# hulop/SfM

Measured on AMD Instinct MI355X. Metric: BA iterations/sec + residual-evals/sec (cams x pts x obs); 1/2/4/8 GPU, higher is better.
Workload: dtype f64; 1 GPU; C3 per GPU: full BA solve (LM + DENSE_SCHUR, Ceres default options); cams=500, points=200000, observations=2000000, points_per_gpu=200000, obs_per_gpu=2000000, views_per_point=10, parallelism=single GPU, reduced_camera_factor=single GPU

## Files before the change

### sfm_amd/csrc/ba_device.h

```cpp
#pragma once
#include <hip/hip_runtime.h>
#include <algorithm>
#include <cstdint>

namespace sfm {

constexpr int kJRec = 20;
constexpr int kJX = 0, kRes = 6, kJC = 8;
constexpr int kEU = 4;
constexpr int kCamR = 36;
constexpr int kUcam = 28;
constexpr int kPtV = 10;
constexpr int kPtL = 10;
constexpr int kPtS = 16;
constexpr int kNB = 64;
constexpr int kThreads = 256;
constexpr uint32_t kYSentinelWord = 0x7FF4DEADu;
constexpr uint64_t kYSentinel = (uint64_t(kYSentinelWord) << 32) | kYSentinelWord;

enum Scalar {
  kCost = 0,
  kGradMaxCam,
  kGradMaxPt,
  kXNorm2Cam,
  kXNorm2Pt,
  kModelChange,
  kNewCost,
  kStep2Pt,
  kStep2Cam,
  kBadStep,
  kCholFail,
  kBadCam,
  kBadBack,
  kModelChangePt,
  kNumScalars
};

struct ReduceJob {
  int slot, nb, op, dst;
};
struct ReduceBatch {
  ReduceJob job[8];
  int n = 0;
  void add(int slot, int nb, int op, int dst) { job[n++] = ReduceJob{slot, nb, op, dst}; }
};

struct DevProblem {
  int32_t C = 0, P = 0;
  int64_t N = 0;
  int32_t* pt_off = nullptr;
  int32_t* order = nullptr;
  int64_t N_pad = 0;
  int32_t* cam_obs = nullptr;
  int32_t* cam_rng = nullptr;
  int32_t* cm_p = nullptr;
  int4* jchunks = nullptr;
  int32_t n_jchunks = 0;
  int32_t xcd_slice_max = 0;
  int32_t* tile_cnt = nullptr;
  int32_t* tile_exp = nullptr;
  int32_t overlap = 0;
  int32_t* jgrp = nullptr;
  int32_t jac_blocks = 1;
  int32_t jac_blocks_rec = 1;
  double* uv_cm = nullptr;
  int32_t* pos = nullptr;
  double* Kc = nullptr;
  double* cam = nullptr;
  double* cam_new = nullptr;
  double* X = nullptr;
  double* X_new = nullptr;
  double* cam0 = nullptr;
  double* X0 = nullptr;
  double* scale_c = nullptr;
  double* scale_p = nullptr;
  double* diag_c = nullptr;
  double* diag_p = nullptr;
  double* camR = nullptr;
  double* camRn = nullptr;
  double* jrec = nullptr;
  double* eu = nullptr;
  bool eu_cm = false;
  double* ypt = nullptr;
  int32_t* wcam = nullptr;
  double* ptV = nullptr;
  double* ptL = nullptr;
  double* Ucam = nullptr;
  int32_t n = 0, ld = 0, nblk = 0;
  double* S = nullptr;
  double* Spack = nullptr;
  double* invL = nullptr;
  double* ysol = nullptr;
  int32_t* fail = nullptr;
  int32_t* flags = nullptr;
  int32_t* cflags = nullptr;
  unsigned long long* cticket = nullptr;
  int32_t n_cu = 0;
  double min_diag = 1e-6, max_diag = 1e32;

  int64_t n_blk = 0, n_pairs = 0;
  int2* blk = nullptr;
  int32_t* seg = nullptr;
  int32_t* bpts = nullptr;
  int32_t* bperm = nullptr;
  int64_t n_bslots = 0;
  double* ptS = nullptr;
  int32_t schur_pts_sub = 8;
  bool schur_wg_blocks = false;
  double* dpart = nullptr;
  double* jpart = nullptr;
  double* uv_pm = nullptr;
  int32_t* cam_pm = nullptr;
  double* partials = nullptr;
  int32_t max_blocks = 0;
  double* scal = nullptr;
  double* scal_host = nullptr;
  const int32_t* gate = nullptr;
  const double* radius_dev = nullptr;
};

enum PartialSlot {
  kPCost = 0, kPXNormCam, kPXNormPt, kPGradCam, kPGradPt, kPModel, kPNewCost, kPStepPt, kPStepCam, kPBad,
  kPBadCam, kPBadBack, kPModelPt,
  kNumPartialSlots
};

void launch_cam_prep(const DevProblem& d, double* cam, bool count_norm, hipStream_t s);
void launch_cam_prep_accept(const DevProblem& d, bool count_norm, int grid, hipStream_t s);
void launch_jacobian(const DevProblem& d, bool scaled, hipStream_t s, bool write_records = false);
void launch_cam_reduce(const DevProblem& d, hipStream_t s);
void launch_cam_finalize(const DevProblem& d, int mode, bool reuse_diag, bool count_grad, hipStream_t s);
void launch_cam_sum_finalize(const DevProblem& d, int mode, bool count_grad, hipStream_t s);
void launch_point_eval(const DevProblem& d, int mode, bool reuse_diag, hipStream_t s);
void launch_point_prep(const DevProblem& d, double radius, hipStream_t s);
void launch_point_factor(const DevProblem& d, double radius, hipStream_t s);
void launch_schur(const DevProblem& d, double radius, bool add_diag, hipStream_t s);
void launch_schur_diag(const DevProblem& d, double radius, bool add_diag, hipStream_t s);
void launch_schur_offdiag(const DevProblem& d, int* tile_cnt, hipStream_t s);
void launch_pad_init(const DevProblem& d, hipStream_t s);
void launch_pack_upper(const DevProblem& d, bool unpack, hipStream_t s);
void launch_gated_copy(const double* src, double* dst, int64_t n, double scale, const int32_t* gate, hipStream_t s);
void launch_cam_update(const DevProblem& d, bool count_norm, hipStream_t s);
bool launch_point_eval_with_cams(const DevProblem& d, int mode, bool count_grad, hipStream_t s);
void launch_point_backsub(const DevProblem& d, hipStream_t s, bool cams_var = true, bool pts_var = true);
inline int obs_xcd_blocks(const DevProblem& d) {
  const int64_t per = d.xcd_slice_max > 0 ? (int64_t(d.xcd_slice_max) + 3) / 4
                                          : ((d.N_pad / 64 + 3) / 4 + 7) / 8;
  return int(8 * std::max<int64_t>(1, per));
}
inline int pt_xcd_blocks(const DevProblem& d) {
  const int64_t per_slice = (int64_t(d.P) + 7) / 8;
  return int(8 * std::max<int64_t>(1, (per_slice + kThreads - 1) / kThreads));
}
void launch_cam_solve(const DevProblem& d, double radius, hipStream_t s);
void launch_reduce(const DevProblem& d, int slot, int nb, int op, int dst, hipStream_t s);
void launch_reduce_batch(const DevProblem& d, const ReduceBatch& b, bool copy_fail, hipStream_t s);
int blocks_for(int64_t n, int threads);

bool launch_cholesky(const DevProblem& d, int epoch, hipStream_t s, bool clear_fail = true, int cam_step = -1,
                     int overlap = 0);
void launch_backsolve(const DevProblem& d, int epoch, hipStream_t s, bool sentinel_set = false);

int launch_cholesky_panel(const DevProblem& d, int k, int pt, int epoch, hipStream_t s);
void launch_panel_update(const DevProblem& d, int k, int j0, int j1, int pt, int nranks, int rank, hipStream_t s);
int panel_update_tiles(int nblk, int pt, int j0, int j1, int nranks, int rank);
constexpr int kPanelPack = 0, kPanelUnpack = 1, kPanelAdd = 2;
void launch_panel_copy(const DevProblem& d, int mode, int pt, int col0, int col1, const int64_t* off, int64_t off1,
                       double* buf, hipStream_t s);
void launch_fail_slot(const DevProblem& d, bool put, double* slot, hipStream_t s);
void launch_spd_fill(double* A, int ld, int n, unsigned seed, hipStream_t s);

}
```

### sfm_amd/csrc/ba_kernels.hip

```cpp
#include <hip/hip_runtime.h>
#include <cfloat>
#include <cmath>
#include <cstdlib>
#include "ba_device.h"
#include "ba_common.h"

namespace sfm {

namespace {

__global__ __launch_bounds__(kThreads) void k_cam_prep(int C, double* __restrict__ cam,
                                                       double* __restrict__ camR, double* __restrict__ part_xn, const int* __restrict__ gate,
                                                       const double* __restrict__ cam_src, const double* __restrict__ X_src,
                                                       double* __restrict__ X_dst, int64_t n_x) {
  if (gate && *gate == 0) return;
  __shared__ double sh[4];
  const int c = blockIdx.x * blockDim.x + threadIdx.x;
  for (int64_t i = int64_t(blockIdx.x) * blockDim.x + threadIdx.x; i < n_x; i += int64_t(gridDim.x) * blockDim.x)
    X_dst[i] = X_src[i];
  if (int64_t(blockIdx.x) * blockDim.x >= C) return;
  double xn = 0.0;
  if (c < C) {
    const double* cs = cam_src ? cam_src : cam;
    double x6[6];
// ... 122 lines not shown
    const double2 uv_nxt = ld2(uv_cm + 2 * (int64_t(ch_n.y) + l));
    const int p_nn = cm_p[int64_t(chunk_at(t + 2).y) + l];
    const double* cr = camR + size_t(kCamR) * c;
    const double* k = Kc + 5 * size_t(c);
    double sc[6];
#pragma unroll
    for (int a = 0; a < 6; ++a) sc[a] = scaled ? scale_c[6 * size_t(c) + a] : 1.0;
    {
      double rec[kJRec];
      const double cl = jac_record(cr, cam[6 * c + 3], cam[6 * c + 4], cam[6 * c + 5], k[0], k[1], k[2], k[3], k[4],
                                   sc, spc, Xc, uv_cur, rec);
      cost += (l < cnt) ? cl : 0.0;
      if (kRec) {
        double* mine = wst + l * kJRec;
#pragma unroll
        for (int f = 0; f < kJRec; f += 2) st2(mine + f, rec[f], rec[f + 1]);
      }
      if (jpart) {
        double j0[6], j1[6], r0 = rec[kRes], r1 = rec[kRes + 1];
#pragma unroll
        for (int a = 0; a < 6; ++a) {
          j0[a] = rec[kJC + a];
          j1[a] = rec[kJC + 6 + a];
        }
        if (cnt < 64) {
          const bool real = l < cnt;
#pragma unroll
          for (int a = 0; a < 6; ++a) {
            j0[a] = real ? j0[a] : 0.0;
            j1[a] = real ? j1[a] : 0.0;
          }
          r0 = real ? r0 : 0.0;
          r1 = real ? r1 : 0.0;
        }
        int q = 0;
#pragma unroll
        for (int a = 0; a < 6; ++a)
#pragma unroll
          for (int b = a; b < 6; ++b, ++q) acc[q] += j0[a] * j0[b] + j1[a] * j1[b];
#pragma unroll
        for (int a = 0; a < 6; ++a) acc[21 + a] += j0[a] * r0 + j1[a] * r1;
        double tot = 0.0;
        if (t + 1 >= n_chunks || ch_n.x != c) {
          tot = wave_sum32(acc, l);
#pragma unroll
          for (int e = 0; e < 32; ++e) acc[e] = 0.0;
        }
        if (!(l & 1) && (l >> 1) < 27) jpart[size_t(ib / 64) * 27 + (l >> 1)] = tot;
      }
    }
    if (kRec) {
      wave_lds_sync();
      jac_flush(wst, jrec, ib, l);
      wave_lds_sync();
    }
#pragma unroll
    for (int j = 0; j < 3; ++j) { Xc[j] = Xn[j]; spc[j] = spn[j]; }
    uv_cur = uv_nxt;
    p_nxt = p_nn;
  }
  const double r = block_reduce(cost, sh, false);
  if (threadIdx.x == 0) part_cost[blockIdx.x] = r;
}

__global__ __launch_bounds__(64) void k_cam_sum(const int32_t* __restrict__ cam_rng,
                                                const double* __restrict__ jpart, double* __restrict__ Ucam, const int* __restrict__ gate) {
  if (gate && *gate == 0) return;
  const int c = blockIdx.x, t = threadIdx.x;
  const int w0 = cam_rng[2 * c] / 64, w1 = (cam_rng[2 * c + 1] + 63) / 64;
  double v[32];
#pragma unroll
  for (int e = 0; e < 32; ++e) v[e] = 0.0;
  for (int w = w0 + t; w < w1; w += 64) {
    const double* src = jpart + size_t(w) * 27;
#pragma unroll
    for (int e = 0; e < 27; ++e) v[e] += src[e];
  }
  const double sum = wave_sum32(v, t);
  if (!(t & 1) && (t >> 1) < 27) Ucam[size_t(kUcam) * c + (t >> 1)] = sum;
}

struct CamFold {
  const int32_t* cam_rng;
  const double* jpart;
  double* Ucam;
  double* scale_c;
  double* diag_c;
  double min_diag, max_diag;
  int mode, C;
  double* part_grad;
};
__device__ __forceinline__ void cam_sum_body(int c, int t, const CamFold& f) {
  const int w0 = f.cam_rng[2 * c] / 64, w1 = (f.cam_rng[2 * c + 1] + 63) / 64;
  double v[32];
#pragma unroll
  for (int e = 0; e < 32; ++e) v[e] = 0.0;
  for (int w = w0 + t; w < w1; w += 64) {
    const double* src = f.jpart + size_t(w) * 27;
#pragma unroll
    for (int e = 0; e < 27; ++e) v[e] += src[e];
  }
  const double sum = wave_sum32(v, t);
  if (!(t & 1) && (t >> 1) < 27) f.Ucam[size_t(kUcam) * c + (t >> 1)] = sum;
  const int a = t < 6 ? t : 0;
  const double cn = __shfl(sum, 2 * up6(a, a)), ga = __shfl(sum, 2 * (21 + a));
  double g = 0.0;
  if (t < 6) {
    if (f.mode == 0) {
      f.scale_c[6 * c + a] = 1.0 / (1.0 + sqrt(cn));
    } else {
      f.diag_c[6 * c + a] = fmin(fmax(cn, f.min_diag), f.max_diag);
      g = fabs(ga / f.scale_c[6 * c + a]);
    }
  }
#pragma unroll
  for (int off = 4; off > 0; off >>= 1) g = fmax(g, __shfl_xor(g, off));
  if (t == 0 && f.part_grad) f.part_grad[c] = g;
}

__global__ __launch_bounds__(64) void k_cam_sum_finalize(const CamFold f, const int* __restrict__ gate) {
  if (gate && *gate == 0) return;
  cam_sum_body(blockIdx.x, threadIdx.x, f);
}

__global__ __launch_bounds__(kThreads) void k_cam_finalize(int C, const double* __restrict__ Ucam,
                                                           double* __restrict__ scale_c, double* __restrict__ diag_c,
                                                           double min_diag, double max_diag, int mode, int reuse,
                                                           double* __restrict__ part_grad, const int* __restrict__ gate) {
  if (gate && *gate == 0) return;
  __shared__ double sh[4];
  const int c = blockIdx.x * blockDim.x + threadIdx.x;
  double g = 0.0;
  if (c < C) {
    const double* U = Ucam + size_t(kUcam) * c;
    for (int a = 0; a < 6; ++a) {
      const double cn = U[up6(a, a)];
      if (mode == 0) {
        scale_c[6 * c + a] = 1.0 / (1.0 + sqrt(cn));
      } else {
        if (!reuse) diag_c[6 * c + a] = fmin(fmax(cn, min_diag), max_diag);
        g = fmax(g, fabs(U[21 + a] / scale_c[6 * c + a]));
      }
    }
  }
  const double r = block_reduce(g, sh, true);
  if (threadIdx.x == 0 && part_grad) part_grad[blockIdx.x] = r;
}

struct CamView {
  const double* R; const double* t; const double* K;
  int sR, sT, sK;
};

__device__ __forceinline__ void point_eval_body(int p, const int32_t* __restrict__ pt_off,
                                                const int32_t* __restrict__ cam_pm,
                                                const double* __restrict__ uv_pm, const CamView cv,
                                                const double* __restrict__ X, double* __restrict__ scale_p,
                                                double* __restrict__ diag_p, double* __restrict__ ptV,
                                                double min_diag, double max_diag, int mode, int reuse, double& g,
                                                double& xn) {
  double V[6] = {0, 0, 0, 0, 0, 0}, b[3] = {0, 0, 0};
  const double Xp[3] = {X[3 * size_t(p)], X[3 * size_t(p) + 1], X[3 * size_t(p) + 2]};
  double sp[3] = {1.0, 1.0, 1.0};
  if (mode == 1)
    for (int k = 0; k < 3; ++k) sp[k] = scale_p[3 * size_t(p) + k];
  const int q0 = pt_off[p], q1 = pt_off[p + 1];
  int c_n = q0 < q1 ? cam_pm[q0] : 0;
  double2 uv_n = q0 < q1 ? ld2(uv_pm + 2 * size_t(q0)) : make_double2(0.0, 0.0);
  for (int q = q0; q < q1; ++q) {
    const int c = c_n;
    const double2 uvo = uv_n;
    if (q + 1 < q1) {
      c_n = cam_pm[q + 1];
      uv_n = ld2(uv_pm + 2 * size_t(q + 1));
    }
    const double* cr = cv.R + size_t(cv.sR) * c;
    const double* k5 = cv.K + size_t(cv.sK) * c;
    const double* tc = cv.t + size_t(cv.sT) * c;
    const double fx = k5[0], sk = k5[1], cx = k5[2], fy = k5[3], cy = k5[4];
    const double pc0 = cr[0] * Xp[0] + cr[1] * Xp[1] + cr[2] * Xp[2] + tc[0];
    const double pc1 = cr[3] * Xp[0] + cr[4] * Xp[1] + cr[5] * Xp[2] + tc[1];
    const double pc2 = cr[6] * Xp[0] + cr[7] * Xp[1] + cr[8] * Xp[2] + tc[2];
    const SharedDiv dz = shared_div(pc2);
    const double xp = sdiv(dz, pc0), yp = sdiv(dz, pc1);
    const double r0 = fx * xp + sk * yp + cx - uvo.x;
    const double r1 = fy * yp + cy - uvo.y;
    const double iz = srcp(dz);
    const double a0 = fx * iz, a1 = sk * iz, a2 = -(fx * xp + sk * yp) * iz;
    const double b1 = fy * iz, b2 = -fy * yp * iz;
    double u[3], v[3];
#pragma unroll
    for (int j = 0; j < 3; ++j) {
      u[j] = (a0 * cr[j] + a1 * cr[3 + j] + a2 * cr[6 + j]) * sp[j];
      v[j] = (b1 * cr[3 + j] + b2 * cr[6 + j]) * sp[j];
    }
    V[0] += u[0] * u[0] + v[0] * v[0];
    V[1] += u[1] * u[0] + v[1] * v[0]; V[2] += u[1] * u[1] + v[1] * v[1];
    V[3] += u[2] * u[0] + v[2] * v[0]; V[4] += u[2] * u[1] + v[2] * v[1]; V[5] += u[2] * u[2] + v[2] * v[2];
    b[0] += u[0] * r0 + v[0] * r1; b[1] += u[1] * r0 + v[1] * r1; b[2] += u[2] * r0 + v[2] * r1;
  }
  const double cn[3] = {V[0], V[2], V[5]};
  if (mode == 0) {
    for (int k = 0; k < 3; ++k) scale_p[3 * size_t(p) + k] = 1.0 / (1.0 + sqrt(cn[k]));
  } else {
    for (int k = 0; k < 3; ++k) {
      if (!reuse) diag_p[3 * size_t(p) + k] = fmin(fmax(cn[k], min_diag), max_diag);
      g = fmax(g, fabs(b[k] / scale_p[3 * size_t(p) + k]));
      xn += X[3 * size_t(p) + k] * X[3 * size_t(p) + k];
    }
    double* o = ptV + size_t(kPtV) * p;
    st2(o, V[0], V[1]); st2(o + 2, V[2], V[3]); st2(o + 4, V[4], V[5]); st2(o + 6, b[0], b[1]); st2(o + 8, b[2], 0.0);
  }
}

__global__ __launch_bounds__(kThreads) void k_point_eval_rc(int P, const int32_t* __restrict__ pt_off,
                                                            const int32_t* __restrict__ cam_pm,
                                                            const double* __restrict__ uv_pm,
                                                            const double* __restrict__ camR,
                                                            const double* __restrict__ cam,
                                                            const double* __restrict__ Kc,
                                                            const double* __restrict__ X,
                                                            double* __restrict__ scale_p, double* __restrict__ diag_p,
                                                            double* __restrict__ ptV, double min_diag, double max_diag,
                                                            int mode, int reuse, double* __restrict__ part_grad,
                                                            double* __restrict__ part_xn, const int* __restrict__ gate) {
  if (gate && *gate == 0) return;
  __shared__ double sh[4];
  const int p = blockIdx.x * blockDim.x + threadIdx.x;
  double g = 0.0, xn = 0.0;
  if (p < P)
    point_eval_body(p, pt_off, cam_pm, uv_pm, CamView{camR, cam + 3, Kc, kCamR, 6, 5}, X, scale_p, diag_p, ptV,
                    min_diag, max_diag, mode, reuse, g, xn);
  if (mode == 1) {
    const double rg = block_reduce(g, sh, true);
    if (threadIdx.x == 0) part_grad[blockIdx.x] = rg;
    const double rx = block_reduce(xn, sh, false);
    if (threadIdx.x == 0) part_xn[blockIdx.x] = rx;
  }
}

constexpr int kCamE = 17;
template <int kMaxC, int kGroups = 1>
__global__ __launch_bounds__(kThreads * kGroups) void k_point_eval_lds(int P, int C, const int32_t* __restrict__ pt_off,
                                                             const int32_t* __restrict__ cam_pm,
                                                             const double* __restrict__ uv_pm,
                                                             const double* __restrict__ camR,
                                                             const double* __restrict__ cam,
                                                             const double* __restrict__ Kc,
                                                             const double* __restrict__ X,
                                                             double* __restrict__ scale_p, double* __restrict__ diag_p,
                                                             double* __restrict__ ptV, double min_diag, double max_diag,
                                                             int mode, int reuse, double* __restrict__ part_grad,
                                                             double* __restrict__ part_xn, const int* __restrict__ gate,
                                                             const CamFold cf) {
  if (gate && *gate == 0) return;
  static_assert(kGroups == 1 || kMaxC > 64, "the camera fold runs with one group per workgroup");
  const int nbp = (P + kThreads - 1) / kThreads;
  if (kGroups == 1 && int(blockIdx.x) >= nbp) {
    const int c = (int(blockIdx.x) - nbp) * (kThreads / 64) + int(threadIdx.x >> 6);
    if (c < cf.C) cam_sum_body(c, threadIdx.x & 63, cf);
    return;
  }
  __shared__ double sh[4 * kGroups];
  __shared__ double cst[kMaxC * kCamE];
  for (int i = threadIdx.x; i < C * kCamE; i += blockDim.x) {
    const int c = i / kCamE, j = i - c * kCamE;
    cst[i] = j < 9 ? camR[size_t(kCamR) * c + j] : j < 12 ? cam[6 * size_t(c) + 3 + (j - 9)] : Kc[5 * size_t(c) + (j - 12)];
  }
  __syncthreads();
  const int grp = int(threadIdx.x) / kThreads, tg = int(threadIdx.x) % kThreads;
  const int vb = int(blockIdx.x) * kGroups + grp;
  const int p = vb * kThreads + tg;
  double g = 0.0, xn = 0.0;
  if (p < P)
    point_eval_body(p, pt_off, cam_pm, uv_pm, CamView{cst, cst + 9, cst + 12, kCamE, kCamE, kCamE}, X, scale_p,
                    diag_p, ptV, min_diag, max_diag, mode, reuse, g, xn);
  if (mode == 1) {
    const int w = int(threadIdx.x) >> 6, l = int(threadIdx.x) & 63;
    const double wg = wave_max(g), wx = wave_sum(xn);
    if (l == 0) sh[w] = wg;
    __syncthreads();
    double rg = 0.0;
    if (tg == 0) {
      rg = sh[4 * grp];
      for (int i = 1; i < 4; ++i) rg = fmax(rg, sh[4 * grp + i]);
    }
    __syncthreads();
    if (l == 0) sh[w] = wx;
    __syncthreads();
    if (tg == 0 && vb < nbp) {
      double rx = sh[4 * grp];
      for (int i = 1; i < 4; ++i) rx = rx + sh[4 * grp + i];
      part_grad[vb] = rg;
      part_xn[vb] = rx;
    }
  }
}

__global__ __launch_bounds__(kThreads) void k_point_factor(int P, const double* __restrict__ ptV,
                                                           const double* __restrict__ diag_p, double radius,
                                                           double* __restrict__ ptL, double* __restrict__ part_bad,
                                                           const double* __restrict__ X,
                                                           const double* __restrict__ scale_p,
                                                           double* __restrict__ ptS, const int* __restrict__ gate, const double* __restrict__ radius_dev) {
  if (gate && *gate == 0) return;
  if (radius_dev) radius = *radius_dev;
  __shared__ double sh[4];
  const int p = blockIdx.x * blockDim.x + threadIdx.x;
  double bad = 0.0;
  if (p < P) {
    const double* v = ptV + size_t(kPtV) * p;
    double D[3];
    for (int k = 0; k < 3; ++k) { const double d = sqrt(diag_p[3 * size_t(p) + k] / radius); D[k] = d * d; }
    const double V00 = v[0] + D[0], V10 = v[1], V11 = v[2] + D[1], V20 = v[3], V21 = v[4], V22 = v[5] + D[2];
    const double l00 = sqrt(V00);
    const double l10 = V10 / l00, l20 = V20 / l00;
    const double l11 = sqrt(V11 - l10 * l10);
    const double l21 = (V21 - l20 * l10) / l11;
    const double l22 = sqrt(V22 - l20 * l20 - l21 * l21);
    if (!(l00 > 0.0) || !(l11 > 0.0) || !(l22 > 0.0)) bad = 1.0;
    const double z0 = v[6] / l00, z1 = (v[7] - l10 * z0) / l11, z2 = (v[8] - l20 * z0 - l21 * z1) / l22;
    double* L = ptL + size_t(kPtL) * p;
    st2(L, l00, l10); st2(L + 2, l11, l20); st2(L + 4, l21, l22); st2(L + 6, z0, z1); st2(L + 8, z2, 0.0);
    if (ptS) {
      double* o = ptS + size_t(kPtS) * p;
      const double* x = X + 3 * size_t(p);
      const double* sp = scale_p + 3 * size_t(p);
      st2(o, x[0], x[1]); st2(o + 2, x[2], sp[0]); st2(o + 4, sp[1], sp[2]);
      st2(o + 6, l10, l20); st2(o + 8, l21, 1.0 / l00); st2(o + 10, 1.0 / l11, 1.0 / l22);
      st2(o + 12, z0, z1); st2(o + 14, z2, 0.0);
    }
  }
  const double r = block_reduce(bad, sh, true);
  if (threadIdx.x == 0) part_bad[blockIdx.x] = r;
}

struct ObsRC {
  double rec[kJRec];
  double M[6];
  double h0, h1;
};
__device__ __forceinline__ void obs_recompute(int c, int p, double2 uvo, const double* __restrict__ camR,
                                              const double* __restrict__ cam, const double* __restrict__ Kc,
                                              const double* __restrict__ scale_c, const double* __restrict__ ptS,
                                              ObsRC& o) {
  const double* cr = camR + size_t(kCamR) * c;
  const double* k = Kc + 5 * size_t(c);
  const double* tc = cam + 6 * size_t(c) + 3;
  const double* sc = scale_c + 6 * size_t(c);
  const double fx = k[0], sk = k[1], cx = k[2], fy = k[3], cy = k[4];
  const double* rp = ptS + size_t(kPtS) * p;
  double q[16];
#pragma unroll
  for (int f = 0; f < 16; f += 2) {
    const double2 x = ld2(rp + f);
    q[f] = x.x; q[f + 1] = x.y;
  }
  const double Xp[3] = {q[0], q[1], q[2]}, sp[3] = {q[3], q[4], q[5]};
  const double pc0 = cr[0] * Xp[0] + cr[1] * Xp[1] + cr[2] * Xp[2] + tc[0];
  const double pc1 = cr[3] * Xp[0] + cr[4] * Xp[1] + cr[5] * Xp[2] + tc[1];
  const double pc2 = cr[6] * Xp[0] + cr[7] * Xp[1] + cr[8] * Xp[2] + tc[2];
  const double iz = srcp(shared_div(pc2)), xp = pc0 * iz, yp = pc1 * iz;
  double* rec = o.rec;
  rec[kRes] = fx * xp + sk * yp + cx - uvo.x;
  rec[kRes + 1] = fy * yp + cy - uvo.y;
  const double a0 = fx * iz, a1 = sk * iz, a2 = -(fx * xp + sk * yp) * iz;
  const double b1 = fy * iz, b2 = -fy * yp * iz;
#pragma unroll
  for (int j = 0; j < 3; ++j) {
    rec[kJX + j] = (a0 * cr[j] + a1 * cr[3 + j] + a2 * cr[6 + j]) * sp[j];
    rec[kJX + 3 + j] = (b1 * cr[3 + j] + b2 * cr[6 + j]) * sp[j];
  }
#pragma unroll
  for (int kk = 0; kk < 3; ++kk) {
    const double* D = cr + 9 + 9 * kk;
    const double q0 = D[0] * Xp[0] + D[1] * Xp[1] + D[2] * Xp[2];
    const double q1 = D[3] * Xp[0] + D[4] * Xp[1] + D[5] * Xp[2];
    const double q2 = D[6] * Xp[0] + D[7] * Xp[1] + D[8] * Xp[2];
    rec[kJC + kk] = (a0 * q0 + a1 * q1 + a2 * q2) * sc[kk];
    rec[kJC + 6 + kk] = (b1 * q1 + b2 * q2) * sc[kk];
  }
  rec[kJC + 3] = a0 * sc[3]; rec[kJC + 4] = a1 * sc[4]; rec[kJC + 5] = a2 * sc[5];
  rec[kJC + 9] = 0.0;        rec[kJC + 10] = b1 * sc[4]; rec[kJC + 11] = b2 * sc[5];
  const double l10 = q[6], l20 = q[7], l21 = q[8], i00 = q[9], i11 = q[10], i22 = q[11];
  const double* e = rec + kJX;
  o.M[0] = e[0] * i00; o.M[1] = (e[1] - l10 * o.M[0]) * i11; o.M[2] = (e[2] - l20 * o.M[0] - l21 * o.M[1]) * i22;
  o.M[3] = e[3] * i00; o.M[4] = (e[4] - l10 * o.M[3]) * i11; o.M[5] = (e[5] - l20 * o.M[3] - l21 * o.M[4]) * i22;
  o.h0 = o.M[0] * q[12] + o.M[1] * q[13] + o.M[2] * q[14];
  o.h1 = o.M[3] * q[12] + o.M[4] * q[13] + o.M[5] * q[14];
}

struct XcdChunks {
  int t, end, stride;
};
__device__ __forceinline__ XcdChunks xcd_chunks(const int32_t* __restrict__ grp_off, int wv) {
  const int grp = blockIdx.x & 7;
  const int nbg = (int(gridDim.x) - 1 - grp) / 8 + 1;
  const int wi = (blockIdx.x >> 3) * (kThreads / 64) + wv;
  return XcdChunks{grp_off[grp] + wi, grp_off[grp + 1], nbg * (kThreads / 64)};
}

__global__ __launch_bounds__(kThreads) void k_obs_prep_rc(const int32_t* __restrict__ grp_off,
                                                          const int4* __restrict__ chunks,
                                                          const int32_t* __restrict__ cm_p,
                                                          const double* __restrict__ uv_cm,
                                                          const int32_t* __restrict__ cam_obs,
                                                          const double* __restrict__ camR,
                                                          const double* __restrict__ cam,
                                                          const double* __restrict__ Kc,
                                                          const double* __restrict__ scale_c,
                                                          const double* __restrict__ ptS,
                                                          double* __restrict__ dpart, const int* __restrict__ gate) {
  if (gate && *gate == 0) return;
  const int l = threadIdx.x & 63, wv = threadIdx.x >> 6;
  const XcdChunks xc = xcd_chunks(grp_off, wave_uniform(wv));
  if (xc.t >= xc.end) return;
  const int4 ch = chunks[xc.t];
  const int64_t i0 = __builtin_amdgcn_readfirstlane(ch.y);
  const int64_t i = i0 + l;
  const int c = __builtin_amdgcn_readfirstlane(ch.x);
  ObsRC o;
  obs_recompute(c, cm_p[i], ld2(uv_cm + 2 * i), camR, cam, Kc, scale_c, ptS, o);
  const double* jc = o.rec + kJC;
  double F[18];
#pragma unroll
  for (int u = 0; u < 6; ++u) {
    F[3 * u] = jc[u] * o.M[0] + jc[6 + u] * o.M[3];
    F[3 * u + 1] = jc[u] * o.M[1] + jc[6 + u] * o.M[4];
    F[3 * u + 2] = jc[u] * o.M[2] + jc[6 + u] * o.M[5];
  }
  double r0 = o.rec[kRes] - o.h0, r1 = o.rec[kRes + 1] - o.h1;
  if (__builtin_amdgcn_readfirstlane(ch.z) < 64) {
    const bool real = cam_obs[i] >= 0;
#pragma unroll
    for (int e = 0; e < 18; ++e) F[e] = real ? F[e] : 0.0;
    r0 = real ? r0 : 0.0;
    r1 = real ? r1 : 0.0;
  }
  double v[32];
  int q = 0;
#pragma unroll
  for (int u = 0; u < 6; ++u)
#pragma unroll
    for (int w = u; w < 6; ++w, ++q)
      v[q] = F[3 * u] * F[3 * w] + F[3 * u + 1] * F[3 * w + 1] + F[3 * u + 2] * F[3 * w + 2];
#pragma unroll
  for (int u = 0; u < 6; ++u) v[21 + u] = jc[u] * r0 + jc[6 + u] * r1;
#pragma unroll
  for (int e = 27; e < 32; ++e) v[e] = 0.0;
  const double tot = wave_sum32(v, l);
  if (!(l & 1) && (l >> 1) < 27) dpart[size_t(i0 / 64) * 27 + (l >> 1)] = tot;
}

__global__ __launch_bounds__(kThreads) void k_backsub_a_rc(const int32_t* __restrict__ grp_off,
                                                           const int4* __restrict__ chunks,
                                                           const int32_t* __restrict__ cm_p,
                                                           const double* __restrict__ uv_cm,
                                                           const int32_t* __restrict__ cam_obs,
                                                           const double* __restrict__ camR,
                                                           const double* __restrict__ cam,
                                                           const double* __restrict__ Kc,
                                                           const double* __restrict__ scale_c,
                                                           const double* __restrict__ ptS,
                                                           const double* __restrict__ ysol, double* __restrict__ eu,
                                                           int eu_cm, double* __restrict__ part_model, const int* __restrict__ gate) {
  if (gate && *gate == 0) return;
  __shared__ double sh[4];
  const int l = threadIdx.x & 63, wv = threadIdx.x >> 6;
  double model = 0.0;
  const XcdChunks xc = xcd_chunks(grp_off, wave_uniform(wv));
  for (int t = xc.t; t < xc.end; t += xc.stride) {
    const int4 ch = chunks[t];
    const int64_t i = int64_t(__builtin_amdgcn_readfirstlane(ch.y)) + l;
    const int c = __builtin_amdgcn_readfirstlane(ch.x);
    ObsRC o;
    obs_recompute(c, cm_p[i], ld2(uv_cm + 2 * i), camR, cam, Kc, scale_c, ptS, o);
    const double* y = ysol + 6 * size_t(c);
    const double* J = o.rec + kJC;
    double e0 = 0.0, e1 = 0.0;
#pragma unroll
    for (int k = 0; k < 6; ++k) { e0 += J[k] * y[k]; e1 += J[6 + k] * y[k]; }
    const int qo = cam_obs[i];
    if (qo >= 0) {
      model += e0 * o.rec[kRes] + e1 * o.rec[kRes + 1] - 0.5 * (e0 * e0 + e1 * e1);
      const double* M = o.M;
      double* dst = eu + 4 * (eu_cm ? size_t(i) : size_t(qo));
      st2(dst, M[0] * e0 + M[3] * e1, M[1] * e0 + M[4] * e1);
      st2(dst + 2, M[2] * e0 + M[5] * e1, 0.0);
    }
  }
  const double r = block_reduce(model, sh, false);
  if (threadIdx.x == 0) part_model[blockIdx.x] = r;
}

__device__ __forceinline__ void schur_diag_body(int c, int C, int t, const int32_t* __restrict__ cam_rng,
                                                const double* __restrict__ dpart, const double* __restrict__ Ucam,
                                                const double* __restrict__ diag_c, double radius, int add_diag,
                                                double* __restrict__ S, int ld, int n, int init,
                                                int* __restrict__ fail, unsigned long long* __restrict__ ysol,
                                                int n_y) {
  for (int j = 6 * c; j < 6 * c + 6; ++j) {
    for (int i = n + 1 + t; i < ld; i += 64) S[size_t(j) * ld + i] = 0.0;
    if (t == 0 && j < n_y) ysol[j] = kYSentinel;
  }
  if (c == C - 1) {
    for (int j = n; j < ld; ++j) {
      for (int i = (j > n ? j : n + 1) + t; i < ld; i += 64) S[size_t(j) * ld + i] = (i == j) ? 1.0 : 0.0;
      if (t == 0 && j < n_y) ysol[j] = kYSentinel;
    }
    if (t == 0) {
      S[size_t(n) * ld + n] = 1.0;
      *fail = 0;
    }
  }
  const int w0 = cam_rng[2 * c] / 64, w1 = (cam_rng[2 * c + 1] + 63) / 64;
  double v[32];
#pragma unroll
  for (int e = 0; e < 32; ++e) v[e] = 0.0;
  for (int w = w0 + t; w < w1; w += 64) {
    const double* src = dpart + size_t(w) * 27;
#pragma unroll
    for (int e = 0; e < 27; ++e) v[e] += src[e];
  }
  const double sum = wave_sum32(v, t);
  const int tu = t < 36 ? t / 6 : 0, tv = t < 36 ? t % 6 : 0;
  const int src = t < 36 ? up6(tu, tv) : (t < 42 ? 21 + (t - 36) : 0);
  const double tot = __shfl(sum, 2 * src);
  if (t < 36) {
    const int u = tu, vv = tv, q = src;
    double* sp = S + size_t(6 * c + u) * ld + 6 * size_t(c) + vv;
    double val = (init ? 0.0 : *sp) - tot;
    if (add_diag) {
      val += Ucam[size_t(kUcam) * c + q];
      if (u == vv) { const double dd = sqrt(diag_c[6 * size_t(c) + u] / radius); val += dd * dd; }
    }
    *sp = val;
  } else if (t < 42) {
    S[size_t(6 * c + (t - 36)) * ld + n] = tot;
  }
}

struct DiagFold {
  const int32_t* cam_rng;
  const double* dpart;
  const double* Ucam;
  const double* diag_c;
  double radius;
  const double* radius_dev;
  int add_diag, C, n, n_y;
  int* fail;
  unsigned long long* ysol;
};

constexpr int kCamS = 50;

__device__ __forceinline__ void stage_cam(double* cs, int c, const double* __restrict__ camR,
                                          const double* __restrict__ cam, const double* __restrict__ Kc,
                                          const double* __restrict__ scale_c, int l) {
  if (l < 36) cs[l] = camR[size_t(kCamR) * c + l];
  else if (l < 39) cs[l] = cam[6 * size_t(c) + 3 + (l - 36)];
  else if (l < 44) cs[l] = Kc[5 * size_t(c) + (l - 39)];
  else if (l < 50) cs[l] = scale_c[6 * size_t(c) + (l - 44)];
}

__device__ __forceinline__ void pair_side_m(const double* cs, const double Xp[3], const double sp[3],
                                            const double Lp[6], double M[6], double ab[5]) {
  const double* cr = cs;
  const double fx = cs[39], sk = cs[40], fy = cs[42];
  const double pc0 = cr[0] * Xp[0] + cr[1] * Xp[1] + cr[2] * Xp[2] + cs[36];
  const double pc1 = cr[3] * Xp[0] + cr[4] * Xp[1] + cr[5] * Xp[2] + cs[37];
  const double pc2 = cr[6] * Xp[0] + cr[7] * Xp[1] + cr[8] * Xp[2] + cs[38];
  const double iz = srcp(shared_div(pc2)), xp = pc0 * iz, yp = pc1 * iz;
  const double a0 = fx * iz, a1 = sk * iz, a2 = -(fx * xp + sk * yp) * iz;
  const double b1 = fy * iz, b2 = -fy * yp * iz;
  ab[0] = a0; ab[1] = a1; ab[2] = a2; ab[3] = b1; ab[4] = b2;
  double e[6];
#pragma unroll
  for (int j = 0; j < 3; ++j) {
    e[j] = (a0 * cr[j] + a1 * cr[3 + j] + a2 * cr[6 + j]) * sp[j];
    e[3 + j] = (b1 * cr[3 + j] + b2 * cr[6 + j]) * sp[j];
  }
  const double l10 = Lp[0], l20 = Lp[1], l21 = Lp[2], i00 = Lp[3], i11 = Lp[4], i22 = Lp[5];
  M[0] = e[0] * i00; M[1] = (e[1] - l10 * M[0]) * i11; M[2] = (e[2] - l20 * M[0] - l21 * M[1]) * i22;
  M[3] = e[3] * i00; M[4] = (e[4] - l10 * M[3]) * i11; M[5] = (e[5] - l20 * M[3] - l21 * M[4]) * i22;
}
template <int kSub>
__device__ __forceinline__ void seg_reduce32(double (&v)[32], int l) {
#pragma unroll
  for (int d = (kSub >= 64 ? 32 : kSub / 2), n = 32; d >= 1 && n > 1; d >>= 1, n >>= 1) {
    const int h = n / 2;
    const uint64_t m = (l & d) ? ~0ull : 0ull;
#pragma unroll
    for (int j = 0; j < h; ++j) {
      const uint64_t a = __builtin_bit_cast(uint64_t, v[j]), b = __builtin_bit_cast(uint64_t, v[h + j]);
      const double keep = __builtin_bit_cast(double, (b & m) | (a & ~m));
      const double send = __builtin_bit_cast(double, (a & m) | (b & ~m));
      v[j] = keep + __shfl_xor(send, d);
    }
  }
  if (kSub == 64) v[0] += __shfl_xor(v[0], 1);
}
template <int kSub>
__device__ __forceinline__ double seg_sum(double v) {
#pragma unroll
  for (int off = kSub / 2; off > 0; off >>= 1) v += __shfl_xor(v, off);
  return v;
}

template <int kSub, int kWpb = 1>
__global__ __launch_bounds__(kThreads, 3) void k_schur_pts(int64_t n_slots, const int2* __restrict__ blk,
                                                        const int32_t* __restrict__ seg,
                                                        const int32_t* __restrict__ bpts,
                                                        const double* __restrict__ ptS,
                                                        const double* __restrict__ camR,
                                                        const double* __restrict__ cam, const double* __restrict__ Kc,
                                                        const double* __restrict__ scale_c, double* __restrict__ S,
                                                        int ld,
                                                        const int32_t* __restrict__ bperm, const int* __restrict__ gate,
                                                        int* __restrict__ tile_cnt, int nbt, const DiagFold df) {
  if (gate && *gate == 0) return;
  static_assert(kWpb == 1 || (kWpb == kThreads / 64 && kSub == 64), "4 waves per block take 64 lanes each");
  constexpr int kPer = 64 / kSub;
  __shared__ __attribute__((aligned(16))) double cst[kThreads / 64][kPer][2 * kCamS];
  const int l = threadIdx.x & 63, wv = threadIdx.x >> 6, g = l / kSub, sl = l % kSub;
  const int64_t wb = kWpb == 1 ? (int64_t(blockIdx.x) * (kThreads / 64) + wv) * kPer : int64_t(blockIdx.x);
  constexpr int kStride = kSub * kWpb;
  const int lane0 = kWpb == 1 ? sl : 64 * wv + sl;
  auto slot_blk = [&](int64_t k) -> int32_t { return k < n_slots ? (bperm ? bperm[k] : int32_t(k)) : -1; };
  const int32_t bs = slot_blk(wb + g);
  const bool own = bs >= 0;
  const int64_t b = own ? bs : 0;
  const int2 cc = blk[b];
  double* cs1 = cst[wv][g];
  double* cs2 = cs1 + kCamS;
#pragma unroll
  for (int q = 0; q < kPer; ++q) {
    const int32_t bq = slot_blk(wb + q);
    const int2 cq = blk[bq >= 0 ? bq : 0];
    stage_cam(cst[wv][q], cq.x, camR, cam, Kc, scale_c, l);
    stage_cam(cst[wv][q] + kCamS, cq.y, camR, cam, Kc, scale_c, l);
  }
  wave_lds_sync();
  if (kWpb > 1 && df.C > 0 && own && cc.x == cc.y && wv == 0) {
    const double radius = df.radius_dev ? *df.radius_dev : df.radius;
    schur_diag_body(cc.x, df.C, l, df.cam_rng, df.dpart, df.Ucam, df.diag_c, radius, df.add_diag, S, ld, df.n, 1,
                    df.fail, df.ysol, df.n_y);
    asm volatile("s_waitcnt vmcnt(0)" ::: "memory");
  }
  const int kb = seg[b], ke = own ? seg[b + 1] : kb;
  double acc[36];
#pragma unroll
  for (int e = 0; e < 36; ++e) acc[e] = 0.0;
  int len = ke - kb;
#pragma unroll
  for (int off = kSub; off < 64; off <<= 1) len = max(len, __shfl_xor(len, off));
  int p_nx = bpts[kb + lane0 < ke ? kb + lane0 : 0];
  for (int k0 = 0; k0 < len; k0 += kStride) {
    asm volatile("" ::: "memory");
    const int k = kb + k0 + lane0;
    const bool valid = k < ke;
    const int p = p_nx;
    p_nx = bpts[k + kStride < ke ? k + kStride : 0];
    const double* r = ptS + size_t(kPtS) * p;
    double q[12];
#pragma unroll
    for (int f = 0; f < 12; f += 2) {
      const double2 x = ld2(r + f);
      q[f] = x.x; q[f + 1] = x.y;
    }
    const double Xp[3] = {q[0], q[1], q[2]}, sp[3] = {q[3], q[4], q[5]};
    const double Lp[6] = {q[6], q[7], q[8], q[9], q[10], q[11]};
    double M1[6], ab1[5], M2[6], ab2[5];
    pair_side_m(cs1, Xp, sp, Lp, M1, ab1);
    pair_side_m(cs2, Xp, sp, Lp, M2, ab2);
    asm volatile("" ::: "memory");
    const double w = valid ? 1.0 : 0.0;
    const double g00 = (M1[0] * M2[0] + M1[1] * M2[1] + M1[2] * M2[2]) * w;
    const double g01 = (M1[0] * M2[3] + M1[1] * M2[4] + M1[2] * M2[5]) * w;
    const double g10 = (M1[3] * M2[0] + M1[4] * M2[1] + M1[5] * M2[2]) * w;
    const double g11 = (M1[3] * M2[3] + M1[4] * M2[4] + M1[5] * M2[5]) * w;
    double H[3][3];
    {
      const double t00 = g00 * ab2[0], t01 = g00 * ab2[1] + g01 * ab2[3], t02 = g00 * ab2[2] + g01 * ab2[4];
      const double t10 = g10 * ab2[0], t11 = g10 * ab2[1] + g11 * ab2[3], t12 = g10 * ab2[2] + g11 * ab2[4];
      H[0][0] = ab1[0] * t00; H[0][1] = ab1[0] * t01; H[0][2] = ab1[0] * t02;
      H[1][0] = ab1[1] * t00 + ab1[3] * t10; H[1][1] = ab1[1] * t01 + ab1[3] * t11; H[1][2] = ab1[1] * t02 + ab1[3] * t12;
      H[2][0] = ab1[2] * t00 + ab1[4] * t10; H[2][1] = ab1[2] * t01 + ab1[4] * t11; H[2][2] = ab1[2] * t02 + ab1[4] * t12;
    }
    double HQ[3][3];
#pragma unroll
    for (int k = 0; k < 3; ++k) {
      const double* D = cs2 + 9 + 9 * k;
      const double q0 = D[0] * Xp[0] + D[1] * Xp[1] + D[2] * Xp[2];
      const double q1 = D[3] * Xp[0] + D[4] * Xp[1] + D[5] * Xp[2];
      const double q2 = D[6] * Xp[0] + D[7] * Xp[1] + D[8] * Xp[2];
#pragma unroll
      for (int i = 0; i < 3; ++i) HQ[i][k] = H[i][0] * q0 + H[i][1] * q1 + H[i][2] * q2;
    }
#pragma unroll
    for (int u = 0; u < 3; ++u) {
      const double* D = cs1 + 9 + 9 * u;
      const double q0 = D[0] * Xp[0] + D[1] * Xp[1] + D[2] * Xp[2];
      const double q1 = D[3] * Xp[0] + D[4] * Xp[1] + D[5] * Xp[2];
      const double q2 = D[6] * Xp[0] + D[7] * Xp[1] + D[8] * Xp[2];
#pragma unroll
      for (int v = 0; v < 3; ++v) {
        acc[6 * u + v] += q0 * HQ[0][v] + q1 * HQ[1][v] + q2 * HQ[2][v];
        acc[6 * u + 3 + v] += q0 * H[0][v] + q1 * H[1][v] + q2 * H[2][v];
      }
    }
#pragma unroll
    for (int u = 0; u < 3; ++u)
#pragma unroll
      for (int v = 0; v < 3; ++v) {
        acc[6 * (3 + u) + v] += HQ[u][v];
        acc[6 * (3 + u) + 3 + v] += H[u][v];
      }
  }
  double v32[32];
#pragma unroll
  for (int e = 0; e < 32; ++e) v32[e] = acc[e];
  seg_reduce32<kSub>(v32, l);
  double t32 = seg_sum<kSub>(acc[32]), t33 = seg_sum<kSub>(acc[33]), t34 = seg_sum<kSub>(acc[34]),
         t35 = seg_sum<kSub>(acc[35]);
  if (kWpb > 1) {
    __shared__ double red[kWpb][36];
    if (!(sl & 1)) red[wv][sl >> 1] = v32[0];
    if (sl == 0) { red[wv][32] = t32; red[wv][33] = t33; red[wv][34] = t34; red[wv][35] = t35; }
    __syncthreads();
    if (wv != 0) return;
    if (!(sl & 1)) {
      double a = red[0][sl >> 1];
#pragma unroll
      for (int q = 1; q < kWpb; ++q) a += red[q][sl >> 1];
      v32[0] = a;
    }
    if (sl < 4) {
      double a = red[0][32 + sl];
#pragma unroll
      for (int q = 1; q < kWpb; ++q) a += red[q][32 + sl];
      if (sl == 0) t32 = a; else if (sl == 1) t33 = a; else if (sl == 2) t34 = a; else t35 = a;
    }
  }
  if (own) {
    double* Sb = S + size_t(6 * cc.x) * ld + 6 * size_t(cc.y);
    const bool add = cc.x == cc.y;
    const double* sc1 = cst[wv][g] + 44;
    const double* sc2 = sc1 + kCamS;
    auto put = [&](int e, double v) {
      double* q = Sb + size_t(e / 6) * ld + e % 6;
      v = v * sc1[e / 6] * sc2[e % 6];
      v = add ? *q - v : -v;
      if (tile_cnt) __hip_atomic_store(q, v, __ATOMIC_RELAXED, __HIP_MEMORY_SCOPE_AGENT);
      else *q = v;
    };
    constexpr int kR = kSub >= 32 ? 1 : 32 / kSub;
    if (kSub == 64) {
      if (!(sl & 1)) put(sl >> 1, v32[0]);
    } else {
#pragma unroll
      for (int r = 0; r < kR; ++r) put(kR * sl + r, v32[r]);
    }
    if (sl < 4) put(32 + sl, sl == 0 ? t32 : sl == 1 ? t33 : sl == 2 ? t34 : t35);
  }
  if (tile_cnt) {
    asm volatile("s_waitcnt vmcnt(0)" ::: "memory");
    if (own && sl == 0) {
      const int r0 = 6 * cc.y, c0 = 6 * cc.x;
      for (int I = r0 / 64; I <= (r0 + 5) / 64; ++I)
        for (int J = c0 / 64; J <= (c0 + 5) / 64; ++J)
          __hip_atomic_fetch_add(tile_cnt + I * nbt + J, 1, __ATOMIC_RELAXED, __HIP_MEMORY_SCOPE_AGENT);
    }
  }
}

template <int kSub, int kHalf>
__global__ __launch_bounds__(kThreads, 4) void k_schur_pts_half(int64_t n_slots, const int2* __restrict__ blk,
                                                             const int32_t* __restrict__ seg,
                                                             const int32_t* __restrict__ bpts,
                                                             const double* __restrict__ ptS,
                                                             const double* __restrict__ camR,
                                                             const double* __restrict__ cam,
                                                             const double* __restrict__ Kc,
                                                             const double* __restrict__ scale_c, double* __restrict__ S,
                                                             int ld, const int32_t* __restrict__ bperm,
                                                             const int* __restrict__ gate) {
  if (gate && *gate == 0) return;
  constexpr int kPer = 64 / kSub;
  __shared__ __attribute__((aligned(16))) double cst[kThreads / 64][kPer][2 * kCamS];
  const int l = threadIdx.x & 63, wv = threadIdx.x >> 6, g = l / kSub, sl = l % kSub;
  const int64_t wb = (int64_t(blockIdx.x) * (kThreads / 64) + wv) * kPer;
  auto slot_blk = [&](int64_t k) -> int32_t { return k < n_slots ? (bperm ? bperm[k] : int32_t(k)) : -1; };
  const int32_t bs = slot_blk(wb + g);
  const bool own = bs >= 0;
  const int64_t b = own ? bs : 0;
  const int2 cc = blk[b];
  double* cs1 = cst[wv][g];
  double* cs2 = cs1 + kCamS;
#pragma unroll
  for (int q = 0; q < kPer; ++q) {
    const int32_t bq = slot_blk(wb + q);
    const int2 cq = blk[bq >= 0 ? bq : 0];
    stage_cam(cst[wv][q], cq.x, camR, cam, Kc, scale_c, l);
    stage_cam(cst[wv][q] + kCamS, cq.y, camR, cam, Kc, scale_c, l);
  }
  wave_lds_sync();
  const int kb = seg[b], ke = own ? seg[b + 1] : kb;
  double acc[18];
#pragma unroll
  for (int e = 0; e < 18; ++e) acc[e] = 0.0;
  int len = ke - kb;
#pragma unroll
  for (int off = kSub; off < 64; off <<= 1) len = max(len, __shfl_xor(len, off));
  int p_nx = bpts[kb + sl < ke ? kb + sl : 0];
  for (int k0 = 0; k0 < len; k0 += kSub) {
    asm volatile("" ::: "memory");
    const int k = kb + k0 + sl;
    const bool valid = k < ke;
    const int p = p_nx;
    p_nx = bpts[k + kSub < ke ? k + kSub : 0];
    const double* r = ptS + size_t(kPtS) * p;
    double q[12];
#pragma unroll
    for (int f = 0; f < 12; f += 2) {
      const double2 x = ld2(r + f);
      q[f] = x.x; q[f + 1] = x.y;
    }
    const double Xp[3] = {q[0], q[1], q[2]}, sp[3] = {q[3], q[4], q[5]};
    const double Lp[6] = {q[6], q[7], q[8], q[9], q[10], q[11]};
    double M1[6], ab1[5], M2[6], ab2[5];
    pair_side_m(cs1, Xp, sp, Lp, M1, ab1);
    pair_side_m(cs2, Xp, sp, Lp, M2, ab2);
    asm volatile("" ::: "memory");
    const double w = valid ? 1.0 : 0.0;
    const double g00 = (M1[0] * M2[0] + M1[1] * M2[1] + M1[2] * M2[2]) * w;
    const double g01 = (M1[0] * M2[3] + M1[1] * M2[4] + M1[2] * M2[5]) * w;
    const double g10 = (M1[3] * M2[0] + M1[4] * M2[1] + M1[5] * M2[2]) * w;
    const double g11 = (M1[3] * M2[3] + M1[4] * M2[4] + M1[5] * M2[5]) * w;
    double H[3][3];
    {
      const double t00 = g00 * ab2[0], t01 = g00 * ab2[1] + g01 * ab2[3], t02 = g00 * ab2[2] + g01 * ab2[4];
      const double t10 = g10 * ab2[0], t11 = g10 * ab2[1] + g11 * ab2[3], t12 = g10 * ab2[2] + g11 * ab2[4];
      H[0][0] = ab1[0] * t00; H[0][1] = ab1[0] * t01; H[0][2] = ab1[0] * t02;
      H[1][0] = ab1[1] * t00 + ab1[3] * t10; H[1][1] = ab1[1] * t01 + ab1[3] * t11; H[1][2] = ab1[1] * t02 + ab1[3] * t12;
      H[2][0] = ab1[2] * t00 + ab1[4] * t10; H[2][1] = ab1[2] * t01 + ab1[4] * t11; H[2][2] = ab1[2] * t02 + ab1[4] * t12;
    }
    double HQ[3][3];
#pragma unroll
    for (int kq = 0; kq < 3; ++kq) {
      const double* D = cs2 + 9 + 9 * kq;
      const double q0 = D[0] * Xp[0] + D[1] * Xp[1] + D[2] * Xp[2];
      const double q1 = D[3] * Xp[0] + D[4] * Xp[1] + D[5] * Xp[2];
      const double q2 = D[6] * Xp[0] + D[7] * Xp[1] + D[8] * Xp[2];
#pragma unroll
      for (int i = 0; i < 3; ++i) HQ[i][kq] = H[i][0] * q0 + H[i][1] * q1 + H[i][2] * q2;
    }
    if (kHalf == 0) {
#pragma unroll
      for (int u = 0; u < 3; ++u) {
        const double* D = cs1 + 9 + 9 * u;
        const double q0 = D[0] * Xp[0] + D[1] * Xp[1] + D[2] * Xp[2];
        const double q1 = D[3] * Xp[0] + D[4] * Xp[1] + D[5] * Xp[2];
        const double q2 = D[6] * Xp[0] + D[7] * Xp[1] + D[8] * Xp[2];
#pragma unroll
        for (int v = 0; v < 3; ++v) {
          acc[6 * u + v] += q0 * HQ[0][v] + q1 * HQ[1][v] + q2 * HQ[2][v];
          acc[6 * u + 3 + v] += q0 * H[0][v] + q1 * H[1][v] + q2 * H[2][v];
        }
      }
    } else {
#pragma unroll
      for (int u = 0; u < 3; ++u)
#pragma unroll
        for (int v = 0; v < 3; ++v) {
          acc[6 * u + v] += HQ[u][v];
          acc[6 * u + 3 + v] += H[u][v];
        }
    }
  }
  double v32[32];
#pragma unroll
  for (int e = 0; e < 32; ++e) v32[e] = e < 18 ? acc[e] : 0.0;
  seg_reduce32<kSub>(v32, l);
  if (own) {
    double* Sb = S + size_t(6 * cc.x) * ld + 6 * size_t(cc.y);
    const bool add = cc.x == cc.y;
    const double* sc1 = cst[wv][g] + 44;
    const double* sc2 = sc1 + kCamS;
    auto put = [&](int e, double v) {
      double* q = Sb + size_t(e / 6) * ld + e % 6;
      v = v * sc1[e / 6] * sc2[e % 6];
      *q = add ? *q - v : -v;
    };
    constexpr int kR = kSub >= 32 ? 1 : 32 / kSub;
    if (kSub == 64) {
      if (!(sl & 1) && (sl >> 1) < 18) put(18 * kHalf + (sl >> 1), v32[0]);
    } else {
#pragma unroll
      for (int r = 0; r < kR; ++r)
        if (kR * sl + r < 18) put(18 * kHalf + kR * sl + r, v32[r]);
    }
  }
}

__global__ __launch_bounds__(64) void k_schur_diag_sum(const int32_t* __restrict__ cam_rng,
                                                       const double* __restrict__ dpart,
                                                       const double* __restrict__ Ucam,
                                                       const double* __restrict__ diag_c, double radius,
                                                       int add_diag, double* __restrict__ S, int ld, int n,
                                                       int init, const int* __restrict__ gate, const double* __restrict__ radius_dev,
                                                       int* __restrict__ fail, unsigned long long* __restrict__ ysol, int n_y) {
  if (gate && *gate == 0) return;
  if (radius_dev) radius = *radius_dev;
  schur_diag_body(blockIdx.x, gridDim.x, threadIdx.x, cam_rng, dpart, Ucam, diag_c, radius, add_diag, S, ld, n, init,
                  fail, ysol, n_y);
}

__device__ __forceinline__ size_t packed_row(int i, int n) { return size_t(i) * (n + 1) - size_t(i) * (i - 1) / 2; }

__global__ void k_pack_upper(const double* __restrict__ S, int ld, int n, double* __restrict__ P, const int* __restrict__ gate) {
  if (gate && *gate == 0) return;
  const int i = blockIdx.x;
  const double* row = S + size_t(i) * ld;
  double* dst = P + packed_row(i, n) - i;
  for (int j = i + threadIdx.x; j <= n; j += blockDim.x) dst[j] = row[j];
}

__global__ void k_unpack_upper(const double* __restrict__ P, int ld, int n, double* __restrict__ S, const int* __restrict__ gate) {
  if (gate && *gate == 0) return;
  const int i = blockIdx.x;
  double* row = S + size_t(i) * ld;
  const double* src = P + packed_row(i, n) - i;
  for (int j = i + threadIdx.x; j <= n; j += blockDim.x) row[j] = src[j];
}

__global__ void k_gated_copy(const double* src, double* dst, int64_t n, double scale, const int* __restrict__ gate) {
  if (gate && *gate == 0) return;
  for (int64_t i = blockIdx.x * int64_t(blockDim.x) + threadIdx.x; i < n; i += int64_t(gridDim.x) * blockDim.x)
    dst[i] = src[i] * scale;
}

__global__ void k_pad_init(double* __restrict__ S, int ld, int n, int* __restrict__ fail,
                           unsigned long long* __restrict__ ysol, int n_y, const int* __restrict__ gate) {
  if (gate && *gate == 0) return;
  const int j = blockIdx.x;
  if (j == 0 && threadIdx.x == 0) *fail = 0;
  if (threadIdx.x == 0 && j < n_y) ysol[j] = kYSentinel;
  for (int i = (j > n ? j : n + 1) + threadIdx.x; i < ld; i += blockDim.x) S[size_t(j) * ld + i] = (i == j) ? 1.0 : 0.0;
  if (j == n && threadIdx.x == 0) S[size_t(n) * ld + n] = 1.0;
}

__global__ __launch_bounds__(kThreads) void k_cam_update(int C, const double* __restrict__ cam,
                                                         const double* __restrict__ ysol,
                                                         const double* __restrict__ scale_c,
                                                         double* __restrict__ cam_new, double* __restrict__ camRn,
                                                         double* __restrict__ part_step, double* __restrict__ part_bad, const int* __restrict__ gate) {
  if (gate && *gate == 0) return;
  __shared__ double sh[4];
  const int c = blockIdx.x * blockDim.x + threadIdx.x;
  double st = 0.0, bad = 0.0;
  if (c < C) cam_update_one(c, cam, ysol, scale_c, cam_new, camRn, st, bad);
  const double rs = block_reduce(st, sh, false);
  if (threadIdx.x == 0 && part_step) part_step[blockIdx.x] = rs;
  const double rb = block_reduce(bad, sh, true);
  if (threadIdx.x == 0) part_bad[blockIdx.x] = rb;
}

__global__ __launch_bounds__(kThreads) void k_cam_solve(int C, const double* __restrict__ Ucam,
                                                        const double* __restrict__ diag_c, double radius,
                                                        double* __restrict__ ysol, int* __restrict__ fail, const int* __restrict__ gate, const double* __restrict__ radius_dev) {
  if (gate && *gate == 0) return;
  if (radius_dev) radius = *radius_dev;
  const int c = blockIdx.x * blockDim.x + threadIdx.x;
  if (c >= C) return;
  const double* U = Ucam + size_t(kUcam) * c;
  double L[21], y[6];
  bool ok = true;
#pragma unroll
  for (int j = 0; j < 6; ++j) {
    double s = U[up6(j, j)] + diag_c[6 * c + j] / radius;
#pragma unroll
    for (int k = 0; k < j; ++k) s -= L[up6(k, j)] * L[up6(k, j)];
    ok = ok && s > 0.0 && isfinite(s);
    const double ljj = sqrt(s);
    L[up6(j, j)] = ljj;
#pragma unroll
    for (int i = j + 1; i < 6; ++i) {
      double a = U[up6(j, i)];
#pragma unroll
      for (int k = 0; k < j; ++k) a -= L[up6(k, i)] * L[up6(k, j)];
      L[up6(j, i)] = a / ljj;
    }
  }
#pragma unroll
  for (int i = 0; i < 6; ++i) {
    double s = U[21 + i];
#pragma unroll
    for (int k = 0; k < i; ++k) s -= L[up6(k, i)] * y[k];
    y[i] = s / L[up6(i, i)];
  }
#pragma unroll
  for (int i = 5; i >= 0; --i) {
    double s = y[i];
#pragma unroll
    for (int k = i + 1; k < 6; ++k) s -= L[up6(i, k)] * y[k];
    y[i] = s / L[up6(i, i)];
  }
#pragma unroll
  for (int i = 0; i < 6; ++i) ysol[6 * c + i] = y[i];
  if (!ok) atomicOr(fail, 1);
}


__global__ __launch_bounds__(kThreads) void k_backsub_b(int P, const int32_t* __restrict__ pt_off,
                                                        const double* __restrict__ eu,
                                                        const int32_t* __restrict__ eu_pos,
                                                        const double* __restrict__ ptL,
                                                        const double* __restrict__ ptV,
                                                        const double* __restrict__ scale_p,
                                                        const double* __restrict__ X, double* __restrict__ X_new,
                                                        double* __restrict__ ypt, double* __restrict__ part_step,
                                                        double* __restrict__ part_bad,
                                                        double* __restrict__ part_model, const int* __restrict__ gate) {
  if (gate && *gate == 0) return;
  __shared__ double sh[4];
  const int x = blockIdx.x & 7;
  const int pb = int((int64_t(x) * P + 7) / 8), pe = int((int64_t(x + 1) * P + 7) / 8);
  const int p = pb + (blockIdx.x >> 3) * blockDim.x + threadIdx.x;
  double st = 0.0, bad = 0.0, model = 0.0;
  if (p < pe) {
    const double* L = ptL + size_t(kPtL) * p;
    const double l00 = L[0], l10 = L[1], l11 = L[2], l20 = L[3], l21 = L[4], l22 = L[5];
    double w0 = L[6], w1 = L[7], w2 = L[8];
    double s0 = 0.0, s1 = 0.0, s2 = 0.0;
    const int q0 = pt_off[p], q1 = pt_off[p + 1];
    int q = q0;
    for (; q + 4 <= q1; q += 4) {
      int ps[4];
#pragma unroll
      for (int j = 0; j < 4; ++j) ps[j] = eu_pos ? eu_pos[q + j] : q + j;
      double2 a[4];
      double b[4];
#pragma unroll
      for (int j = 0; j < 4; ++j) {
        const double* u = eu + 4 * size_t(ps[j]);
        a[j] = ld2(u);
        b[j] = u[2];
      }
#pragma unroll
      for (int j = 0; j < 4; ++j) {
        w0 -= a[j].x;
        w1 -= a[j].y;
        w2 -= b[j];
        s0 += a[j].x; s1 += a[j].y; s2 += b[j];
      }
    }
    for (; q < q1; ++q) {
      const double* u = eu + 4 * (eu_pos ? size_t(eu_pos[q]) : size_t(q));
      const double2 u01 = ld2(u);
      const double u2 = u[2];
      w0 -= u01.x;
      w1 -= u01.y;
      w2 -= u2;
      s0 += u01.x; s1 += u01.y; s2 += u2;
    }
    const double y2 = w2 / l22;
    const double y1 = (w1 - l21 * y2) / l11;
    const double y0 = (w0 - l10 * y1 - l20 * y2) / l00;
    if (!isfinite(y0) || !isfinite(y1) || !isfinite(y2)) bad = 1.0;
    {
      const double* v = ptV + size_t(kPtV) * p;
      const double h0 = l00 * s0, h1 = l10 * s0 + l11 * s1, h2 = l20 * s0 + l21 * s1 + l22 * s2;
      const double yVy = v[0] * y0 * y0 + v[2] * y1 * y1 + v[5] * y2 * y2 +
                         2.0 * (v[1] * y0 * y1 + v[3] * y0 * y2 + v[4] * y1 * y2);
      model = y0 * (v[6] - h0) + y1 * (v[7] - h1) + y2 * (v[8] - h2) - 0.5 * yVy;
    }
    const double yp[3] = {y0, y1, y2};
    for (int k = 0; k < 3; ++k) {
      const double x = X[3 * size_t(p) + k];
      const double xn = x + scale_p[3 * size_t(p) + k] * (-yp[k]);
      const double d = x - xn;
      st += d * d;
      X_new[3 * size_t(p) + k] = xn;
      ypt[3 * size_t(p) + k] = yp[k];
    }
  }
  double r = block_reduce(st, sh, false);
  if (threadIdx.x == 0) part_step[blockIdx.x] = r;
  r = block_reduce(bad, sh, true);
  if (threadIdx.x == 0) part_bad[blockIdx.x] = r;
  r = block_reduce(model, sh, false);
  if (threadIdx.x == 0) part_model[blockIdx.x] = r;
}

__global__ __launch_bounds__(kThreads) void k_backsub_c(const int32_t* __restrict__ grp_off,
                                                        const int4* __restrict__ chunks,
                                                        const int32_t* __restrict__ cam_obs,
                                                        const int32_t* __restrict__ cm_p,
                                                        const double* __restrict__ uv_cm,
                                                        const double* __restrict__ Kc,
                                                        const double* __restrict__ X_new,
                                                        const double* __restrict__ camRn,
                                                        double* __restrict__ part_cost, const int* __restrict__ gate) {
  if (gate && *gate == 0) return;
  __shared__ double sh[4];
  const int l = threadIdx.x & 63, wv = threadIdx.x >> 6;
  const XcdChunks xc = xcd_chunks(grp_off, wave_uniform(wv));
  double ncost = 0.0;
  if (xc.t < xc.end) {
    const int4 ch = chunks[xc.t];
    const int64_t i = int64_t(__builtin_amdgcn_readfirstlane(ch.y)) + l;
    const int c = __builtin_amdgcn_readfirstlane(ch.x);
    const bool real = cam_obs[i] >= 0;
    const int p = cm_p[i];
    const double* Rn = camRn + 12 * size_t(c);
    const double Xn0 = X_new[3 * size_t(p)], Xn1 = X_new[3 * size_t(p) + 1], Xn2 = X_new[3 * size_t(p) + 2];
    double pc[3];
#pragma unroll
    for (int k = 0; k < 3; ++k) pc[k] = Rn[3 * k] * Xn0 + Rn[3 * k + 1] * Xn1 + Rn[3 * k + 2] * Xn2 + Rn[9 + k];
    const SharedDiv dz = shared_div(pc[2]);
    const double xp = sdiv(dz, pc[0]), ypj = sdiv(dz, pc[1]);
    const double* k5 = Kc + 5 * size_t(c);
    const double2 uvo = ld2(uv_cm + 2 * i);
    const double rn0 = k5[0] * xp + k5[1] * ypj + k5[2] - uvo.x;
    const double rn1 = k5[3] * ypj + k5[4] - uvo.y;
    if (real) ncost = 0.5 * (rn0 * rn0 + rn1 * rn1);
  }
  const double r = block_reduce(ncost, sh, false);
  if (threadIdx.x == 0) part_cost[blockIdx.x] = r;
}

__global__ __launch_bounds__(1024) void k_reduce_batch(const double* __restrict__ partials, int64_t max_blocks,
                                                       ReduceBatch b, double* __restrict__ scal,
                                                       const int* __restrict__ fail, const int* __restrict__ gate) {
  if (gate && *gate == 0) return;
  __shared__ double sh[16];
  reduce_batch_job(partials, max_blocks, b.job[blockIdx.x], scal, blockIdx.x == 0 ? fail : nullptr, sh);
}

__global__ __launch_bounds__(1024) void k_reduce(const double* __restrict__ src, int nb, int op,
                                                 double* __restrict__ dst) {
  __shared__ double sh[16];
  double v = 0.0;
  for (int i = threadIdx.x; i < nb; i += 1024) v = op ? fmax(v, src[i]) : v + src[i];
  v = op ? wave_max(v) : wave_sum(v);
  const int w = threadIdx.x >> 6, l = threadIdx.x & 63;
  if (l == 0) sh[w] = v;
  __syncthreads();
  if (threadIdx.x == 0) {
    double r = sh[0];
    for (int i = 1; i < 16; ++i) r = op ? fmax(r, sh[i]) : r + sh[i];
    *dst = r;
  }
}

}

int blocks_for(int64_t n, int threads) { return int((n + threads - 1) / threads); }

static inline double* slot(const DevProblem& d, int s) { return d.partials + size_t(s) * d.max_blocks; }

void launch_cam_prep(const DevProblem& d, double* cam, bool count_norm, hipStream_t s) {
  k_cam_prep<<<blocks_for(d.C, kThreads), kThreads, 0, s>>>(d.C, cam, d.camR, count_norm ? slot(d, kPXNormCam) : nullptr, d.gate,
                                                            nullptr, nullptr, nullptr, 0);
}
void launch_cam_prep_accept(const DevProblem& d, bool count_norm, int grid, hipStream_t s) {
  k_cam_prep<<<std::max(grid, blocks_for(d.C, kThreads)), kThreads, 0, s>>>(
      d.C, d.cam, d.camR, count_norm ? slot(d, kPXNormCam) : nullptr, d.gate, d.cam_new, d.X_new, d.X, 3 * int64_t(d.P));
}
void launch_jacobian(const DevProblem& d, bool scaled, hipStream_t s, bool write_records) {
  if (write_records)
    k_jacobian<true><<<d.jac_blocks_rec, kThreads, 0, s>>>(d.jgrp, d.jchunks, d.cm_p, d.uv_cm, d.Kc, d.cam, d.camR,
                                                           d.X, d.scale_c, d.scale_p, scaled ? 1 : 0, d.jrec,
                                                           slot(d, kPCost), d.jpart, d.gate);
  else
    k_jacobian<false><<<d.jac_blocks, kThreads, 0, s>>>(d.jgrp, d.jchunks, d.cm_p, d.uv_cm, d.Kc, d.cam, d.camR, d.X,
                                                        d.scale_c, d.scale_p, scaled ? 1 : 0, d.jrec, slot(d, kPCost),
                                                        d.jpart, d.gate);
}
void launch_cam_reduce(const DevProblem& d, hipStream_t s) {
  if (d.C) k_cam_sum<<<d.C, 64, 0, s>>>(d.cam_rng, d.jpart, d.Ucam, d.gate);
}
static CamFold cam_fold(const DevProblem& d, int mode, bool count_grad) {
  return CamFold{d.cam_rng, d.jpart, d.Ucam, d.scale_c, d.diag_c, d.min_diag, d.max_diag, mode, d.C,
                 count_grad ? slot(d, kPGradCam) : nullptr};
}
void launch_cam_sum_finalize(const DevProblem& d, int mode, bool count_grad, hipStream_t s) {
  if (d.C) k_cam_sum_finalize<<<d.C, 64, 0, s>>>(cam_fold(d, mode, count_grad), d.gate);
}
bool launch_point_eval_with_cams(const DevProblem& d, int mode, bool count_grad, hipStream_t s) {
  if (d.P == 0 || d.C == 0 || d.C > 64) return false;
  const int nb = blocks_for(d.P, kThreads) + (d.C + kThreads / 64 - 1) / (kThreads / 64);
  k_point_eval_lds<64><<<nb, kThreads, 0, s>>>(d.P, d.C, d.pt_off, d.cam_pm, d.uv_pm, d.camR, d.cam, d.Kc, d.X,
                                               d.scale_p, d.diag_p, d.ptV, d.min_diag, d.max_diag, mode, 0,
                                               slot(d, kPGradPt), slot(d, kPXNormPt), d.gate,
                                               cam_fold(d, mode, count_grad));
  return true;
}
void launch_cam_finalize(const DevProblem& d, int mode, bool reuse_diag, bool count_grad, hipStream_t s) {
  k_cam_finalize<<<blocks_for(d.C, kThreads), kThreads, 0, s>>>(d.C, d.Ucam, d.scale_c, d.diag_c, d.min_diag, d.max_diag, mode,
                                                               reuse_diag ? 1 : 0,
                                                               count_grad ? slot(d, kPGradCam) : nullptr, d.gate);
}
static bool env_flag_k(const char* name) {
  const char* v = std::getenv(name);
  return v && v[0] == '1';
}
void launch_point_eval(const DevProblem& d, int mode, bool reuse_diag, hipStream_t s) {
  if (d.P == 0) return;
  const int nb = blocks_for(d.P, kThreads);
#define SFM_PE_LDS(M_)                                                                                              \
  k_point_eval_lds<M_><<<nb, kThreads, 0, s>>>(d.P, d.C, d.pt_off, d.cam_pm, d.uv_pm, d.camR, d.cam, d.Kc, d.X,      \
                                               d.scale_p, d.diag_p, d.ptV, d.min_diag, d.max_diag, mode,           \
                                               reuse_diag ? 1 : 0, slot(d, kPGradPt), slot(d, kPXNormPt), d.gate,    \
                                               CamFold{})
  if (d.C <= 64) SFM_PE_LDS(64);
  else if (d.C <= 512 && !env_flag_k("SFM_PE_GROUPS1"))
    k_point_eval_lds<512, 2><<<blocks_for(d.P, 2 * kThreads), 2 * kThreads, 0, s>>>(
        d.P, d.C, d.pt_off, d.cam_pm, d.uv_pm, d.camR, d.cam, d.Kc, d.X, d.scale_p, d.diag_p, d.ptV, d.min_diag,
        d.max_diag, mode, reuse_diag ? 1 : 0, slot(d, kPGradPt), slot(d, kPXNormPt), d.gate, CamFold{});
  else if (d.C <= 512) SFM_PE_LDS(512);
  else
    k_point_eval_rc<<<nb, kThreads, 0, s>>>(d.P, d.pt_off, d.cam_pm, d.uv_pm, d.camR, d.cam, d.Kc, d.X, d.scale_p,
                                            d.diag_p, d.ptV, d.min_diag, d.max_diag, mode, reuse_diag ? 1 : 0,
                                            slot(d, kPGradPt), slot(d, kPXNormPt), d.gate);
#undef SFM_PE_LDS
}
void launch_point_factor(const DevProblem& d, double radius, hipStream_t s) {
  if (d.P) k_point_factor<<<blocks_for(d.P, kThreads), kThreads, 0, s>>>(d.P, d.ptV, d.diag_p, radius, d.ptL,
                                                                         slot(d, kPBad), d.X, d.scale_p, d.ptS, d.gate, d.radius_dev);
}
void launch_point_prep(const DevProblem& d, double radius, hipStream_t s) {
  launch_point_factor(d, radius, s);
  if (d.N_pad)
    k_obs_prep_rc<<<obs_xcd_blocks(d), kThreads, 0, s>>>(d.jgrp, d.jchunks, d.cm_p, d.uv_cm, d.cam_obs, d.camR, d.cam,
                                                         d.Kc, d.scale_c, d.ptS, d.dpart, d.gate);
}
void launch_schur(const DevProblem& d, double radius, bool add_diag, hipStream_t s) {
  if (d.schur_wg_blocks && d.n_blk && d.C) {
    const DiagFold f{d.cam_rng, d.dpart, d.Ucam, d.diag_c, radius, d.radius_dev, add_diag ? 1 : 0, d.C, d.n,
                     (d.n + kNB - 1) / kNB * kNB, d.fail, reinterpret_cast<unsigned long long*>(d.ysol)};
    k_schur_pts<64, kThreads / 64><<<int(d.n_bslots), kThreads, 0, s>>>(d.n_bslots, d.blk, d.seg, d.bpts, d.ptS,
                                                                       d.camR, d.cam, d.Kc, d.scale_c, d.S, d.ld,
                                                                       d.bperm, d.gate, nullptr, d.nblk, f);
    return;
  }
  launch_schur_diag(d, radius, add_diag, s);
  launch_schur_offdiag(d, nullptr, s);
}
void launch_schur_diag(const DevProblem& d, double radius, bool add_diag, hipStream_t s) {
  if (d.C)
    k_schur_diag_sum<<<d.C, 64, 0, s>>>(d.cam_rng, d.dpart, d.Ucam, d.diag_c, radius, add_diag ? 1 : 0, d.S, d.ld,
                                        d.n, 1, d.gate, d.radius_dev, d.fail,
                                        reinterpret_cast<unsigned long long*>(d.ysol), (d.n + kNB - 1) / kNB * kNB);
}
void launch_schur_offdiag(const DevProblem& d, int* tile_cnt, hipStream_t s) {
  if (!d.n_blk) return;
  const int64_t n_slots = tile_cnt ? d.n_blk : d.n_bslots;
  const int32_t* bperm = tile_cnt ? nullptr : d.bperm;
  const int sub = d.schur_pts_sub, per = 64 / sub * (kThreads / 64);
  const int nb = int((n_slots + per - 1) / per);
#define SFM_PTS(S_)                                                                                           \
  k_schur_pts<S_><<<nb, kThreads, 0, s>>>(n_slots, d.blk, d.seg, d.bpts, d.ptS, d.camR, d.cam, d.Kc, d.scale_c, \
                                          d.S, d.ld, bperm, d.gate, tile_cnt, d.nblk, DiagFold{})
  if (d.schur_wg_blocks) {
    k_schur_pts<64, kThreads / 64><<<int(n_slots), kThreads, 0, s>>>(n_slots, d.blk, d.seg, d.bpts, d.ptS,
                                                                    d.camR, d.cam, d.Kc, d.scale_c, d.S, d.ld,
                                                                    bperm, d.gate, tile_cnt, d.nblk, DiagFold{});
    return;
  }
  static const bool halves = [] {
    const char* e = std::getenv("SFM_SCHUR_HALVES");
    return e && e[0] == '1';
  }();
  if (halves && !tile_cnt) {
#define SFM_PTS_H(S_, H_)                                                                                       \
  k_schur_pts_half<S_, H_><<<nb, kThreads, 0, s>>>(n_slots, d.blk, d.seg, d.bpts, d.ptS, d.camR, d.cam, d.Kc, \
                                                   d.scale_c, d.S, d.ld, bperm, d.gate)
    if (sub == 8) { SFM_PTS_H(8, 0); SFM_PTS_H(8, 1); }
    else if (sub == 16) { SFM_PTS_H(16, 0); SFM_PTS_H(16, 1); }
    else if (sub == 32) { SFM_PTS_H(32, 0); SFM_PTS_H(32, 1); }
    else { SFM_PTS_H(64, 0); SFM_PTS_H(64, 1); }
#undef SFM_PTS_H
    return;
  }
  if (sub == 8) SFM_PTS(8);
  else if (sub == 16) SFM_PTS(16);
  else if (sub == 32) SFM_PTS(32);
  else SFM_PTS(64);
#undef SFM_PTS
}
void launch_pack_upper(const DevProblem& d, bool unpack, hipStream_t s) {
  if (d.n == 0) return;
  if (unpack) k_unpack_upper<<<d.n, 256, 0, s>>>(d.Spack, d.ld, d.n, d.S, d.gate);
  else k_pack_upper<<<d.n, 256, 0, s>>>(d.S, d.ld, d.n, d.Spack, d.gate);
}
void launch_gated_copy(const double* src, double* dst, int64_t n, double scale, const int32_t* gate, hipStream_t s) {
  if (n <= 0) return;
  const int grid = int(std::min<int64_t>(1024, (n + 255) / 256));
  k_gated_copy<<<grid, 256, 0, s>>>(src, dst, n, scale, gate);
}
void launch_pad_init(const DevProblem& d, hipStream_t s) {
  const int n_y = (d.n + kNB - 1) / kNB * kNB;
  k_pad_init<<<d.ld, 64, 0, s>>>(d.S, d.ld, d.n, d.fail, reinterpret_cast<unsigned long long*>(d.ysol), n_y, d.gate);
}
void launch_cam_update(const DevProblem& d, bool count_norm, hipStream_t s) {
  k_cam_update<<<blocks_for(d.C, kThreads), kThreads, 0, s>>>(d.C, d.cam, d.ysol, d.scale_c, d.cam_new, d.camRn,
                                                             count_norm ? slot(d, kPStepCam) : nullptr,
                                                             slot(d, kPBadCam), d.gate);
}
void launch_cam_solve(const DevProblem& d, double radius, hipStream_t s) {
  (void)hipMemsetAsync(d.fail, 0, sizeof(int), s);
  if (d.C) k_cam_solve<<<blocks_for(d.C, kThreads), kThreads, 0, s>>>(d.C, d.Ucam, d.diag_c, radius, d.ysol, d.fail, d.gate, d.radius_dev);
}
void launch_point_backsub(const DevProblem& d, hipStream_t s, bool cams_var, bool pts_var) {
  if (d.N_pad && cams_var)
    k_backsub_a_rc<<<obs_xcd_blocks(d), kThreads, 0, s>>>(d.jgrp, d.jchunks, d.cm_p, d.uv_cm, d.cam_obs, d.camR,
                                                          d.cam, d.Kc, d.scale_c, d.ptS, d.ysol, d.eu, d.eu_cm ? 1 : 0,
                                                          slot(d, kPModel), d.gate);
  else if (d.N_pad) {
    (void)hipMemsetAsync(d.eu, 0, sizeof(double) * 4 * size_t(d.eu_cm ? d.N_pad : d.N), s);
    (void)hipMemsetAsync(slot(d, kPModel), 0, sizeof(double) * size_t(obs_xcd_blocks(d)), s);
  }
  if (d.P && pts_var) {
    k_backsub_b<<<pt_xcd_blocks(d), kThreads, 0, s>>>(d.P, d.pt_off, d.eu, d.eu_cm ? d.pos : nullptr,
                                                               d.ptL, d.ptV, d.scale_p,
                                                               d.X, d.X_new, d.ypt, slot(d, kPStepPt),
                                                               slot(d, kPBadBack), slot(d, kPModelPt), d.gate);
  } else if (d.P) {
    const size_t nbP = size_t(pt_xcd_blocks(d));
    (void)hipMemsetAsync(d.ypt, 0, sizeof(double) * 3 * size_t(d.P), s);
    (void)hipMemcpyAsync(d.X_new, d.X, sizeof(double) * 3 * size_t(d.P), hipMemcpyDeviceToDevice, s);
    (void)hipMemsetAsync(slot(d, kPStepPt), 0, sizeof(double) * nbP, s);
    (void)hipMemsetAsync(slot(d, kPBadBack), 0, sizeof(double) * nbP, s);
    (void)hipMemsetAsync(slot(d, kPModelPt), 0, sizeof(double) * nbP, s);
  }
  if (d.N_pad)
    k_backsub_c<<<obs_xcd_blocks(d), kThreads, 0, s>>>(d.jgrp, d.jchunks, d.cam_obs, d.cm_p, d.uv_cm, d.Kc, d.X_new,
                                                       d.camRn, slot(d, kPNewCost), d.gate);
}
void launch_reduce(const DevProblem& d, int sl, int nb, int op, int dst, hipStream_t s) {
  k_reduce<<<1, 1024, 0, s>>>(slot(d, sl), nb, op, d.scal + dst);
}
void launch_reduce_batch(const DevProblem& d, const ReduceBatch& b, bool copy_fail, hipStream_t s) {
  if (b.n > 0)
    k_reduce_batch<<<b.n, 1024, 0, s>>>(d.partials, d.max_blocks, b, d.scal, copy_fail ? d.fail : nullptr, d.gate);
}

}
```

### sfm_amd/csrc/ba_solver.hip

```cpp
#include <hip/hip_runtime.h>
#include <rccl/rccl.h>
#include <map>
#include <atomic>
#include <thread>

#include <algorithm>
#include <array>
#include <cfloat>
#include <cmath>
#include <cstdio>
#include <cstdlib>
#include <cstring>
#include <limits>
#include <string>
#include <vector>
#include <chrono>

#include "sfm_trace.h"
#include "ba_device.h"
#include "ba_setup.h"
#include "ba_common.h"
#include "ba_host_layout.h"
#include "../../include/sfm_amd.h"

// ... 573 lines not shown
  for (int J = 0; J < np; ++J) {
    const int c0 = J * pt * kNB, c1 = std::min((J + 1) * pt * kNB, d.n + 1);
    D.count[J] = c1 > c0 ? int64_t(c1 - c0) * (d.n + 1 - c0) : 0;
    D.poff[J] = D.total;
    D.total += D.count[J];
    D.bcast_cap = std::max<int64_t>(D.bcast_cap, D.count[J] + int64_t(pt) * kNB * kNB + 1);
  }
  std::vector<int64_t> os(static_cast<size_t>(np));
  for (int J = 0; J < np; ++J) os[J] = J % N == h->rank ? -1 : D.poff[J];
  auto grab = [&](void** p, size_t bytes) { return hipMalloc(p, std::max<size_t>(bytes, 256)) == hipSuccess; };
  if (!grab(reinterpret_cast<void**>(&D.send), sizeof(double) * size_t(D.total)) ||
      !grab(reinterpret_cast<void**>(&D.recv), sizeof(double) * size_t(D.total)) ||
      !grab(reinterpret_cast<void**>(&D.bcast), 2 * sizeof(double) * size_t(D.bcast_cap)) ||
      !grab(reinterpret_cast<void**>(&D.off_send), sizeof(int64_t) * np))
    return fail(SFM_ENOMEM, "hipMalloc failed (distributed factor buffers)");
  HIPCHK(hipMemcpy(D.off_send, os.data(), sizeof(int64_t) * np, hipMemcpyHostToDevice));
  HIPCHK(hipMemsetAsync(D.send, 0, sizeof(double) * size_t(D.total), h->stream));
  while (int(D.ev_red.size()) < np) {
    hipEvent_t e;
    HIPCHK(hipEventCreateWithFlags(&e, hipEventDisableTiming));
    D.ev_red.push_back(e);
  }
  if (!D.ev_sent) HIPCHK(hipEventCreateWithFlags(&D.ev_sent, hipEventDisableTiming));
  D.pt = pt; D.nblk = d.nblk; D.n = d.n; D.nranks = N; D.rank = h->rank;
  return 0;
}

int dist_factor_enqueue(sfm_ba_handle* h) {
  SFM_TRACE("sfm:dist_factor");
  DevProblem& d = h->d;
  hipStream_t s = h->stream;
  int rc;
  if ((rc = dist_prepare(h))) return rc;
  auto& D = h->dist;
  const int pt = D.pt, N = h->nranks, me = h->rank, np = int(D.count.size());
  static const bool force_overlap = env_flag("SFM_DIST_OVERLAP");
  const bool overlap = h->comm != nullptr && force_overlap;
  const bool comm = N > 1 || overlap;
  hipStream_t cs = overlap ? D.cstream : s;
  launch_panel_copy(d, kPanelPack, pt, 0, d.n + 1, D.off_send, 0, D.send, s);
  if (overlap) {
    HIPCHK(hipEventRecord(D.ev_sent, s));
    HIPCHK(hipStreamWaitEvent(cs, D.ev_sent, 0));
    HIPCHK(hipEventRecord(D.ev_free[0], s));
    HIPCHK(hipEventRecord(D.ev_free[1], s));
  }
  auto reduce_panel = [&](int k) -> int {
    if (!comm || k >= np) return 0;
    if (int e = reduce_to(h, D.send + D.poff[k], D.recv + D.poff[k], D.count[k], k % N, cs)) return e;
    if (overlap && k % N == me) HIPCHK(hipEventRecord(D.ev_red[k], cs));
    return 0;
  };
  auto geom = [&](int k, int* t0, int* c0, int* c1, int64_t* nw) {
    *t0 = k * pt;
    const int ncols = std::min(pt, d.nblk - *t0);
    *c0 = *t0 * kNB;
    *c1 = *c0 + ncols * kNB;
    *nw = int64_t(ncols) * kNB * kNB;
  };
  auto half = [&](int k) { return D.bcast + size_t(k & 1) * size_t(D.bcast_cap); };
  auto factor_pack = [&](int k) -> int {
    int t0, c0, c1;
    int64_t nw;
    geom(k, &t0, &c0, &c1, &nw);
    if (comm) {
      if (overlap) HIPCHK(hipStreamWaitEvent(s, D.ev_red[k], 0));
      launch_panel_copy(d, kPanelAdd, pt, c0, c1, nullptr, D.poff[k], D.recv, s);
    }
    double* b = half(k);
    launch_cholesky_panel(d, k, pt, ++h->chol_epoch, s);
    launch_panel_copy(d, kPanelPack, pt, c0, c1, nullptr, 0, b, s);
    HIPCHK(hipMemcpyAsync(b + D.count[k], d.invL + size_t(t0) * kNB * kNB, sizeof(double) * size_t(nw),
                          hipMemcpyDeviceToDevice, s));
    launch_fail_slot(d, true, b + D.count[k] + nw, s);
    if (overlap) HIPCHK(hipEventRecord(D.ev_packed, s));
    return 0;
  };
  if ((rc = reduce_panel(0)) || (rc = reduce_panel(1))) return rc;
  if (np > 0 && me == 0 && (rc = factor_pack(0))) return rc;
  for (int k = 0; k < np; ++k) {
    const int owner = k % N;
    int t0, c0, c1;
    int64_t nw;
    geom(k, &t0, &c0, &c1, &nw);
    double* b = half(k);
    const int64_t cnt = D.count[k] + nw + 1;
    if (comm) {
      if (overlap) {
        if (me == owner) HIPCHK(hipStreamWaitEvent(cs, D.ev_packed, 0));
        else HIPCHK(hipStreamWaitEvent(cs, D.ev_free[k & 1], 0));
        NCCLCHK(ncclBroadcast(b, b, size_t(cnt), ncclDouble, owner, h->comm, cs));
        HIPCHK(hipEventRecord(D.ev_arrived[k & 1], cs));
      } else if ((rc = broadcast(h, b, cnt, owner))) {
        return rc;
      }
      if ((rc = reduce_panel(k + 2))) return rc;
      if (overlap) HIPCHK(hipStreamWaitEvent(s, D.ev_arrived[k & 1], 0));
    }
    if (me != owner) {
      launch_panel_copy(d, kPanelUnpack, pt, c0, c1, nullptr, 0, b, s);
      HIPCHK(hipMemcpyAsync(d.invL + size_t(t0) * kNB * kNB, b + D.count[k], sizeof(double) * size_t(nw),
                            hipMemcpyDeviceToDevice, s));
      launch_fail_slot(d, false, b + D.count[k] + nw, s);
      if (overlap) HIPCHK(hipEventRecord(D.ev_free[k & 1], s));
    }
    if (k + 1 < np && (k + 1) % N == me) {
      launch_panel_update(d, k, k + 1, k + 1, pt, N, me, s);
      if ((rc = factor_pack(k + 1))) return rc;
    }
    launch_panel_update(d, k, k + 2, INT32_MAX / 2, pt, N, me, s);
  }
  return 0;
}

int fetch_scalars(sfm_ba_handle* h) {
  HIPCHK(hipMemcpyAsync(h->d.scal_host, h->d.scal, sizeof(double) * (kNumScalars + 1), hipMemcpyDeviceToHost,
                        h->stream));
  HIPCHK(hipStreamSynchronize(h->stream));
  collect_marks(h);
  return 0;
}

void reduce_phase(sfm_ba_handle* h, const ReduceBatch& rb, bool copy_fail, int tail) {
  DevProblem& d = h->d;
  if (h->fuse_lm && rb.n > 0) {
#define SFM_RB_LM(T_)                                                                                      \
  k_reduce_batch_lm<T_><<<rb.n, 1024, 0, h->stream>>>(d.partials, d.max_blocks, rb, d.scal,                 \
                                                      copy_fail ? d.fail : nullptr, d.gate, h->lm_ctl,      \
                                                      h->lm_trace, h->lm_trace_cap, af)
    AcceptFold af{};
    if (tail == kTailPost) SFM_RB_LM(kTailPost);
    else if (tail == kTailInit) SFM_RB_LM(kTailInit);
    else {
      if (h->accept_fold)
        af = AcceptFold{d.C, 3 * int64_t(d.P), d.cam, d.camR,
                        h->mode != SFM_BA_STRUCT_ONLY ? d.partials + size_t(kPXNormCam) * d.max_blocks : nullptr,
                        d.cam_new, d.X_new, d.X};
      SFM_RB_LM(kTailDecide);
    }
#undef SFM_RB_LM
    return;
  }
  launch_reduce_batch(d, rb, copy_fail, h->stream);
}

int evaluate_enqueue(sfm_ba_handle* h, bool first, bool jacobi_scaling) {
  SFM_TRACE("sfm:evaluate");
  DevProblem& d = h->d;
  hipStream_t s = h->stream;
  int rc;
  const bool cams_var = h->mode != SFM_BA_STRUCT_ONLY, pts_var = h->mode != SFM_BA_POSE_ONLY;
  const int nbP = std::max(1, blocks_for(d.P, 256)),
            nbC = std::max(1, blocks_for(d.C, 256));
  if (h->accept_grid > 0) launch_cam_prep_accept(d, cams_var, h->accept_grid, s);
  else if (h->accept_grid == 0) launch_cam_prep(d, d.cam, cams_var, s);
  mark_begin(h, kPhJac);
  launch_jacobian(d, !first || !jacobi_scaling ? true : false, s);
  mark_end(h);
  const bool fuse_cam = !sharded(h);
  const bool fold_cams = fuse_cam && cams_var && pts_var && d.P > 0 && d.C > 0 && d.C <= 64;
  if (first && jacobi_scaling) {
    if (fold_cams) {
      mark_begin(h, kPhPtEval);
      launch_point_eval_with_cams(d, 0, false, s);
      mark_end(h);
    } else {
      if (cams_var) {
        mark_begin(h, kPhCamRed);
        if (fuse_cam) {
          launch_cam_sum_finalize(d, 0, false, s);
        } else {
          launch_cam_reduce(d, s);
          if ((rc = allreduce(h, d.Ucam, size_t(kUcam) * d.C, ncclSum))) return rc;
          launch_cam_finalize(d, 0, false, false, s);
        }
        mark_end(h);
      }
      if (pts_var) launch_point_eval(d, 0, false, s);
    }
    mark_begin(h, kPhJac);
    launch_jacobian(d, true, s);
    mark_end(h);
  }
  if (fold_cams) {
    mark_begin(h, kPhPtEval);
    launch_point_eval_with_cams(d, 1, true, s);
    mark_end(h);
  } else if (cams_var) {
    mark_begin(h, kPhCamRed);
    if (fuse_cam) {
      launch_cam_sum_finalize(d, 1, true, s);
    } else {
      launch_cam_reduce(d, s);
      if ((rc = allreduce(h, d.Ucam, size_t(kUcam) * d.C, ncclSum))) return rc;
      launch_cam_finalize(d, 1, false, true, s);
    }
    mark_end(h);
  } else {
    hipMemsetAsync(d.partials + size_t(kPGradCam) * d.max_blocks, 0, sizeof(double) * nbC, s);
    hipMemsetAsync(d.partials + size_t(kPXNormCam) * d.max_blocks, 0, sizeof(double) * nbC, s);
  }
  if (fold_cams) {
  } else if (pts_var) {
    mark_begin(h, kPhPtEval);
    launch_point_eval(d, 1, false, s);
    mark_end(h);
  } else {
    hipMemsetAsync(d.partials + size_t(kPGradPt) * d.max_blocks, 0, sizeof(double) * nbP, s);
    hipMemsetAsync(d.partials + size_t(kPXNormPt) * d.max_blocks, 0, sizeof(double) * nbP, s);
  }
  if (d.N == 0) hipMemsetAsync(d.partials + size_t(kPCost) * d.max_blocks, 0, sizeof(double), s);
  if (d.P == 0) {
    hipMemsetAsync(d.partials + size_t(kPGradPt) * d.max_blocks, 0, sizeof(double), s);
    hipMemsetAsync(d.partials + size_t(kPXNormPt) * d.max_blocks, 0, sizeof(double), s);
  }
  ReduceBatch rb;
  rb.add(kPCost, d.jac_blocks, 0, kCost);
  rb.add(kPGradCam, cams_var && fuse_cam ? std::max(1, d.C) : nbC, 1, kGradMaxCam);
  rb.add(kPGradPt, nbP, 1, kGradMaxPt);
  rb.add(kPXNormCam, nbC, 0, kXNorm2Cam);
  rb.add(kPXNormPt, nbP, 0, kXNorm2Pt);
  reduce_phase(h, rb, false, first ? kTailInit : kTailPost);
  if (sharded(h)) {
    if ((rc = allreduce(h, d.scal + kCost, 1, ncclSum))) return rc;
    if ((rc = allreduce(h, d.scal + kGradMaxCam, 2, ncclMax))) return rc;
    if ((rc = allreduce(h, d.scal + kXNorm2Pt, 1, ncclSum))) return rc;
  }
  return 0;
}
int evaluate(sfm_ba_handle* h, bool first, bool jacobi_scaling) {
  if (int rc = evaluate_enqueue(h, first, jacobi_scaling)) return rc;
  return fetch_scalars(h);
}

int compute_step_enqueue(sfm_ba_handle* h, double radius) {
  SFM_TRACE("sfm:compute_step");
  DevProblem& d = h->d;
  hipStream_t s = h->stream;
  int rc;
  const int nbP = std::max(1, blocks_for(d.P, 256)), nbC = std::max(1, blocks_for(d.C, 256));
  bool cam_done = false;
  if (h->mode == SFM_BA_STRUCT_AND_POSE && d.overlap && d.C && !sharded(h) && !h->force_pack) {
    mark_begin(h, kPhPtPrep);
    launch_point_prep(d, radius, s);
    mark_end(h);
    if (!h->stream2) {
      HIPCHK(hipStreamCreateWithFlags(&h->stream2, hipStreamNonBlocking));
      HIPCHK(hipEventCreateWithFlags(&h->ov_ev[0], hipEventDisableTiming));
      HIPCHK(hipEventCreateWithFlags(&h->ov_ev[1], hipEventDisableTiming));
    }
    const int m_schur = mark_begin(h, kPhSchur);
    HIPCHK(hipMemsetAsync(d.tile_cnt, 0, sizeof(int32_t) * size_t(d.nblk) * d.nblk, s));
    launch_schur_diag(d, radius, h->rank == 0, s);
    HIPCHK(hipEventRecord(h->ov_ev[0], s));
    HIPCHK(hipStreamWaitEvent(h->stream2, h->ov_ev[0], 0));
    mark_begin(h, kPhChol, h->stream2);
    launch_cholesky(d, ++h->chol_epoch, h->stream2, false, -1, d.overlap);
    mark_end(h, h->stream2);
    launch_schur_offdiag(d, d.tile_cnt, s);
    HIPCHK(hipEventRecord(h->ov_ev[1], h->stream2));
    HIPCHK(hipStreamWaitEvent(s, h->ov_ev[1], 0));
    mark_end(h, nullptr, m_schur);
    mark_begin(h, kPhBack);
    launch_backsolve(d, ++h->bs_epoch, s, true);
    mark_end(h);
  } else if (h->mode == SFM_BA_STRUCT_AND_POSE) {
    mark_begin(h, kPhPtPrep);
    launch_point_prep(d, radius, s);
    mark_end(h);
    mark_begin(h, kPhSchur);
    launch_schur(d, radius, h->rank == 0, s);
    mark_end(h);
    if (!d.C) launch_pad_init(d, s);
    if (sharded(h) && h->dist_pt > 0) {
      mark_begin(h, kPhChol);
      if ((rc = dist_factor_enqueue(h))) return rc;
      mark_end(h);
    } else {
      if (sharded(h) || h->force_pack) {
        launch_pack_upper(d, false, s);
        if ((rc = allreduce(h, d.Spack, packed_size(d.n), ncclSum))) return rc;
        launch_pack_upper(d, true, s);
      }
      mark_begin(h, kPhChol);
      cam_done = launch_cholesky(d, ++h->chol_epoch, s, false, h->rank == 0 ? 1 : 0);
      mark_end(h);
    }
    mark_begin(h, kPhBack);
    launch_backsolve(d, ++h->bs_epoch, s, true);
    mark_end(h);
  } else if (h->mode == SFM_BA_POSE_ONLY) {
    launch_cam_solve(d, radius, s);
    if (d.P) launch_point_factor(d, radius, s);
    hipMemsetAsync(d.partials + size_t(kPBad) * d.max_blocks, 0, sizeof(double) * nbP, s);
  } else {
    hipMemsetAsync(d.fail, 0, sizeof(int), s);
    if (d.P) {
      mark_begin(h, kPhPtPrep);
      launch_point_factor(d, radius, s);
      mark_end(h);
    }
    hipMemsetAsync(d.ysol, 0, sizeof(double) * 6 * size_t(d.C), s);
  }
  if (!cam_done) launch_cam_update(d, h->rank == 0 && h->mode != SFM_BA_STRUCT_ONLY, s);
  mark_begin(h, kPhBacksub);
  launch_point_backsub(d, s, h->mode != SFM_BA_STRUCT_ONLY, h->mode != SFM_BA_POSE_ONLY);
  mark_end(h);
  if (d.P == 0) {
    const int slots[] = {kPModel, kPModelPt, kPNewCost, kPStepPt, kPBadBack, kPBad};
    for (int sl : slots) hipMemsetAsync(d.partials + size_t(sl) * d.max_blocks, 0, sizeof(double), s);
  }
  if (h->rank != 0 || h->mode == SFM_BA_STRUCT_ONLY)
    hipMemsetAsync(d.partials + size_t(kPStepCam) * d.max_blocks, 0, sizeof(double) * nbC, s);
  const int nbI = d.N_pad ? obs_xcd_blocks(d) : 1;
  const int nbB = d.P ? pt_xcd_blocks(d) : 1;
  ReduceBatch rb;
  rb.add(kPModel, nbI, 0, kModelChange);
  rb.add(kPNewCost, nbI, 0, kNewCost);
  rb.add(kPStepPt, nbB, 0, kStep2Pt);
  rb.add(kPStepCam, nbC, 0, kStep2Cam);
  rb.add(kPBad, nbP, 1, kBadStep);
  rb.add(kPBadCam, nbC, 1, kBadCam);
  rb.add(kPBadBack, nbB, 1, kBadBack);
  rb.add(kPModelPt, nbB, 0, kModelChangePt);
  reduce_phase(h, rb, true, kTailDecide);
  if (sharded(h)) {
    if ((rc = allreduce(h, d.scal + kModelChange, 4, ncclSum))) return rc;
    if ((rc = allreduce(h, d.scal + kBadStep, 4, ncclMax))) return rc;
    if ((rc = allreduce(h, d.scal + kModelChangePt, 1, ncclSum))) return rc;
  }
  return 0;
}
int compute_step(sfm_ba_handle* h, double radius) {
  if (int rc = compute_step_enqueue(h, radius)) return rc;
  return fetch_scalars(h);
}

const char* invalid_option(const sfm_ba_options& o) {
  if (!(o.max_num_iterations >= 0)) return "max_num_iterations >= 0";
  if (!(o.max_num_consecutive_invalid_steps >= 0)) return "max_num_consecutive_invalid_steps >= 0";
  if (!(o.function_tolerance >= 0)) return "function_tolerance >= 0";
  if (!(o.gradient_tolerance >= 0)) return "gradient_tolerance >= 0";
  if (!(o.parameter_tolerance >= 0)) return "parameter_tolerance >= 0";
  if (!(o.initial_trust_region_radius > 0)) return "initial_trust_region_radius > 0";
  if (!(o.min_trust_region_radius > 0)) return "min_trust_region_radius > 0";
  if (!(o.max_trust_region_radius > 0)) return "max_trust_region_radius > 0";
  if (!(o.min_trust_region_radius <= o.max_trust_region_radius)) return "min_trust_region_radius <= max";
  if (!(o.min_trust_region_radius <= o.initial_trust_region_radius)) return "min_trust_region_radius <= initial";
  if (!(o.initial_trust_region_radius <= o.max_trust_region_radius)) return "initial_trust_region_radius <= max";
  if (!(o.min_relative_decrease >= 0)) return "min_relative_decrease >= 0";
  if (!(o.min_lm_diagonal >= 0)) return "min_lm_diagonal >= 0";
  if (!(o.max_lm_diagonal >= 0)) return "max_lm_diagonal >= 0";
  if (!(o.min_lm_diagonal <= o.max_lm_diagonal)) return "min_lm_diagonal <= max_lm_diagonal";
  return nullptr;
}

template <class Push>
int run_device_lm(sfm_ba_handle* h, const sfm_ba_options& opts, double* cost, sfm_ba_summary* sm, Push& push,
                  bool* nonfinite) {
  DevProblem& d = h->d;
  hipStream_t s = h->stream;
  HostTimer timer;
  timer.tag = "solve";
  if (!h->lm_ctl) {
    if (hipMalloc(reinterpret_cast<void**>(&h->lm_ctl), sizeof(LmCtl)) != hipSuccess) {
      h->lm_ctl = nullptr;
      return fail(SFM_ENOMEM, "hipMalloc failed (LM control)");
    }
    if (hipHostMalloc(reinterpret_cast<void**>(&h->lm_ctl_host), sizeof(LmCtl)) != hipSuccess) {
      h->lm_ctl_host = nullptr;
      return fail(SFM_ENOMEM, "hipHostMalloc failed (LM control)");
    }
  }
  const int cap = std::max(1, opts.max_num_iterations + 1);
  if (h->lm_trace_cap < cap) {
    if (h->lm_trace) {
      (void)hipStreamSynchronize(s);
      (void)hipHostFree(h->lm_trace);
    }
    h->lm_trace = nullptr;
    h->lm_trace_cap = 0;
    if (hipHostMalloc(reinterpret_cast<void**>(&h->lm_trace), sizeof(sfm_ba_iteration) * size_t(cap)) != hipSuccess) {
      h->lm_trace = nullptr;
      return fail(SFM_ENOMEM, "hipMalloc failed (LM trace)");
    }
    h->lm_trace_cap = cap;
  }
  LmCtl& c = *h->lm_ctl_host;
  std::memset(&c, 0, sizeof(c));
  c.run_step = 1;
  c.radius = opts.initial_trust_region_radius;
  c.decrease_factor = 2.0;
  c.max_iter = opts.max_num_iterations;
  c.max_invalid = opts.max_num_consecutive_invalid_steps;
  c.ftol = opts.function_tolerance;
  c.gtol = opts.gradient_tolerance;
  c.ptol = opts.parameter_tolerance;
  c.max_radius = opts.max_trust_region_radius;
  c.min_radius = opts.min_trust_region_radius;
  c.min_rel_dec = opts.min_relative_decrease;
  HIPCHK(hipMemcpyAsync(h->lm_ctl, &c, sizeof(LmCtl), hipMemcpyHostToDevice, s));
  int batch = 3, batch_next = 2;
  if (const char* b = std::getenv("SFM_LM_BATCH")) batch = batch_next = std::max(1, std::min(64, std::atoi(b)));
  if (opts.max_num_iterations <= 0) batch = 0;
  const bool jac_scaling = opts.jacobi_scaling != 0;
  const int acc_blocks = std::max(1, std::min(1024, blocks_for(6 * int64_t(d.C) + 3 * int64_t(d.P), 256)));
  d.radius_dev = &h->lm_ctl->radius;
  h->fuse_lm = !sharded(h) && !env_flag("SFM_LM_UNFUSED");
  h->accept_fold = h->fuse_lm && d.C > 0 && d.C <= kAcceptFoldMaxCams && 3 * int64_t(d.P) <= kAcceptFoldMaxX &&
                   !env_flag("SFM_NO_ACCEPT_FOLD");
  d.gate = nullptr;
  int rc = evaluate_enqueue(h, true, jac_scaling);
  if (rc == 0 && !h->fuse_lm) k_lm_init<<<1, 1, 0, s>>>(h->lm_ctl, d.scal);
  while (rc == 0) {
    for (int b = 0; b < batch && rc == 0; ++b) {
      d.gate = &h->lm_ctl->run_step;
      if ((rc = compute_step_enqueue(h, c.radius))) break;
      d.gate = nullptr;
      if (!h->fuse_lm) k_lm_decide<<<1, 1, 0, s>>>(h->lm_ctl, d.scal, h->lm_trace, h->lm_trace_cap);
      d.gate = &h->lm_ctl->run_eval;
      h->accept_grid = h->accept_fold ? -1 : acc_blocks;
      rc = evaluate_enqueue(h, false, jac_scaling);
      h->accept_grid = 0;
      if (rc) break;
      d.gate = nullptr;
      if (!h->fuse_lm) k_lm_post<<<1, 1, 0, s>>>(h->lm_ctl, d.scal, h->lm_trace, h->lm_trace_cap);
    }
    if (rc) break;
    timer.mark("batch enqueued");
    if (h->prefetch_params) {
      if (hipMemcpyAsync(h->param_host, d.cam, sizeof(double) * 6 * size_t(d.C), hipMemcpyDeviceToHost, s) != hipSuccess ||
          hipMemcpyAsync(h->param_host + 6 * size_t(d.C), d.X, sizeof(double) * 3 * size_t(d.P), hipMemcpyDeviceToHost,
                         s) != hipSuccess) {
        rc = fail(SFM_EIO, "parameter readback failed");
        break;
      }
    }
    if (hipMemcpyAsync(&c, h->lm_ctl, sizeof(LmCtl), hipMemcpyDeviceToHost, s) != hipSuccess ||
        hipStreamSynchronize(s) != hipSuccess) {
      rc = fail(SFM_EIO, "LM control readback failed");
      break;
    }
    timer.mark("batch synchronised");
    collect_marks(h);
    if (c.done) break;
    batch = batch_next;
  }
  d.gate = nullptr;
  d.radius_dev = nullptr;
  h->fuse_lm = false;
  h->accept_fold = false;
  if (rc) return rc;
  if (c.error & 4) return fail(SFM_EIO, "Cholesky tile hand-off timed out (persistent grid made no progress)");
  if (c.error & 2) return fail(SFM_EIO, "back-substitution hand-off timed out (persistent grid made no progress)");
  sm->num_jacobian_evaluations++;
  sm->num_residual_evaluations++;
  sm->initial_cost = c.init_cost;
  if (c.error & 8) {
    *nonfinite = true;
    sm->termination_type = SFM_FAILURE;
    sm->final_cost = c.init_cost;
    return fail(SFM_EIO, "initial residual evaluation is not finite");
  }
  {
    sfm_ba_iteration it0;
    std::memset(&it0, 0, sizeof(it0));
    it0.cost = c.init_cost;
    it0.gradient_max_norm = c.init_grad;
    it0.trust_region_radius = opts.initial_trust_region_radius;
    it0.step_is_valid = 1;
    it0.step_is_successful = 1;
    push(it0);
  }
  const int n_tr = std::min(c.trace_len, h->lm_trace_cap);
  for (int i = 0; i < n_tr; ++i) push(h->lm_trace[i]);
  h->param_host_valid = h->prefetch_params;
  sm->termination_type = c.termination;
  sm->num_iterations = c.iteration;
  sm->num_successful_steps += c.n_succ;
  sm->num_unsuccessful_steps += c.n_unsucc;
  sm->num_invalid_steps += c.n_invalid;
  sm->num_residual_evaluations += c.n_resid;
  sm->num_jacobian_evaluations += c.n_jac;
  sm->num_linear_solves += c.n_lin;
  *cost = c.cost;
  return 0;
}

}

extern "C" {

int32_t sfm_abi_version(void) { return SFM_ABI_VERSION; }
const char* sfm_last_error(void) { return g_err.c_str(); }

void sfm_ba_default_options(sfm_ba_options* o) {
  o->max_num_iterations = 50;
  o->max_num_consecutive_invalid_steps = 5;
  o->jacobi_scaling = 1;
  o->reserved0 = 0;
  o->function_tolerance = 1e-6;
  o->gradient_tolerance = 1e-10;
  o->parameter_tolerance = 1e-8;
  o->initial_trust_region_radius = 1e4;
  o->max_trust_region_radius = 1e16;
  o->min_trust_region_radius = 1e-32;
  o->min_lm_diagonal = 1e-6;
  o->max_lm_diagonal = 1e32;
  o->min_relative_decrease = 1e-3;
}

int32_t sfm_device_count(void) {
  int n = 0;
  if (hipGetDeviceCount(&n) != hipSuccess) return 0;
  return n;
}

int sfm_ba_create(int32_t device, sfm_ba_handle** out) {
  if (!out) return fail(SFM_EINVAL, "out is NULL");
  int n = 0;
  if (hipGetDeviceCount(&n) != hipSuccess || n == 0) return fail(SFM_ENODEV, "no HIP device visible");
  if (device < 0 || device >= n) return fail(SFM_EINVAL, "device ordinal out of range");
  HIPCHK(hipSetDevice(device));
  auto* h = new sfm_ba_handle();
  h->device = device;
  if (hipStreamCreateWithFlags(&h->stream, hipStreamNonBlocking) != hipSuccess) {
    delete h;
    return fail(SFM_EIO, "hipStreamCreate failed");
  }
  h->n_cu = device_cus(device);
  *out = h;
  return 0;
}

int sfm_ba_destroy(sfm_ba_handle* h) {
  if (!h) return 0;
  hipSetDevice(h->device);
  hipStreamSynchronize(h->stream);
  free_problem(h);
  release_pool(h);
  if (h->d.scal_host) hipHostFree(h->d.scal_host);
  if (h->lm_ctl) hipFree(h->lm_ctl);
  if (h->lm_ctl_host) hipHostFree(h->lm_ctl_host);
  if (h->lm_trace) hipHostFree(h->lm_trace);
  if (h->param_host) hipHostFree(h->param_host);
  if (h->stage) hipHostFree(h->stage);
  if (h->ar_tmp) hipFree(h->ar_tmp);
  for (void* p : {static_cast<void*>(h->dist.send), static_cast<void*>(h->dist.recv),
                  static_cast<void*>(h->dist.bcast), static_cast<void*>(h->dist.off_send),
                  static_cast<void*>(h->dist.off_recv)})
    if (p) hipFree(p);
  if (h->dist.cstream) {
    hipStreamSynchronize(h->dist.cstream);
    hipStreamDestroy(h->dist.cstream);
    for (hipEvent_t e : {h->dist.ev_packed, h->dist.ev_free[0], h->dist.ev_free[1], h->dist.ev_arrived[0],
                         h->dist.ev_arrived[1]})
      hipEventDestroy(e);
  }
  for (hipEvent_t e : h->dist.ev_red) hipEventDestroy(e);
  if (h->dist.ev_sent) hipEventDestroy(h->dist.ev_sent);
  if (h->stream2) {
    hipStreamSynchronize(h->stream2);
    hipStreamDestroy(h->stream2);
    hipEventDestroy(h->ov_ev[0]);
    hipEventDestroy(h->ov_ev[1]);
  }
  if (h->ustream) {
    hipStreamSynchronize(h->ustream);
    hipStreamDestroy(h->ustream);
    hipEventDestroy(h->uev);
    if (h->uev_uv) hipEventDestroy(h->uev_uv);
  }
  for (auto e : h->ev) hipEventDestroy(e);
  if (h->comm) ncclCommDestroy(h->comm);
  hipStreamDestroy(h->stream);
  delete h;
  return 0;
}

int sfm_comm_unique_id(uint8_t out[128]) {
  ncclUniqueId id;
  NCCLCHK(ncclGetUniqueId(&id));
  static_assert(sizeof(ncclUniqueId) == 128, "ncclUniqueId size");
  std::memcpy(out, &id, 128);
  return 0;
}

int sfm_ba_set_comm(sfm_ba_handle* h, int32_t nranks, int32_t rank, const uint8_t id[128]) {
  if (!h || nranks < 1 || rank < 0 || rank >= nranks) return fail(SFM_EINVAL, "bad communicator arguments");
  HIPCHK(hipSetDevice(h->device));
  if (h->comm) { ncclCommDestroy(h->comm); h->comm = nullptr; }
  h->host_fn = nullptr;
  h->coll_fn = nullptr;
  h->nranks = nranks;
  h->rank = rank;
  ncclUniqueId uid;
  std::memcpy(&uid, id, 128);
  NCCLCHK(ncclCommInitRank(&h->comm, nranks, uid, rank));
  h->emulate_ranks = 1;
  if (const char* e = std::getenv("SFM_EMULATE_IDENTICAL_RANKS")) h->emulate_ranks = std::max(1, std::atoi(e));
  return 0;
}

int sfm_ba_set_host_comm(sfm_ba_handle* h, int32_t nranks, int32_t rank, sfm_allreduce_fn fn, void* user) {
  if (!h || nranks < 1 || rank < 0 || rank >= nranks || !fn) return fail(SFM_EINVAL, "bad communicator arguments");
  if (h->comm) { ncclCommDestroy(h->comm); h->comm = nullptr; }
  h->nranks = nranks;
  h->rank = rank;
  h->host_fn = fn;
  h->host_user = user;
  h->coll_fn = nullptr;
  h->coll_user = nullptr;
  return 0;
}

namespace {
int coll_as_allreduce(double* buf, int64_t count, int32_t op, void* user) {
  auto* h = static_cast<sfm_ba_handle*>(user);
// ... 185 lines not shown
    {
      Fill32Set fs;
      fs.add(err, 4 * sizeof(int32_t), uint32_t(INT32_MAX));
      fs.add(cnt_c, sizeof(int32_t) * (size_t(C) + 1), 0);
      fs.add(cnt_p, sizeof(int32_t) * (size_t(P) + 1), 0);
      launch_fill32(fs, s);
    }
    launch_validate(N, deferred_uv ? nullptr : in_uv, in_cam, in_pt, C, P, err, cnt_c, deferred_uv ? nullptr : cnt_p, s);
    HCHK(hipMemcpyAsync(stg, err, sizeof(int32_t) * (size_t(C) + 4), hipMemcpyDeviceToHost, s));
    HCHK(hipStreamSynchronize(s));
    std::memcpy(cam_cnt.data(), stg, sizeof(int32_t) * (size_t(C) + 4));
    if (deferred_uv && std::min(cam_cnt[0], cam_cnt[1]) != INT32_MAX) {
      if ((rc = wait_uv())) return bail(rc);
      launch_validate(N, in_uv, in_cam, in_pt, C, P, err, cnt_c, cnt_p, s);
      HCHK(hipMemcpyAsync(stg, err, sizeof(int32_t) * 4, hipMemcpyDeviceToHost, s));
      HCHK(hipStreamSynchronize(s));
      std::memcpy(cam_cnt.data(), stg, sizeof(int32_t) * 4);
    }
  }
  timer.mark("upload + validate");
  {
    const int32_t e0 = cam_cnt[0], e1 = cam_cnt[1], e2 = cam_cnt[2];
    const int32_t first = std::min({e0, e1, e2});
    if (first != INT32_MAX) {
      const char* what = first == e0 ? "cam_idx out of range at " : first == e1 ? "pt_idx out of range at "
                                                                                   : "non-finite observation at ";
      return bail(fail(SFM_EINVAL, what + std::to_string(first)));
    }
  }
  hostlayout::Runs runs;
  hostlayout::camera_runs(C, cam_cnt.data() + 4, &runs);
  const std::vector<int32_t>&cam_off = runs.cam_off, &cam_rng = runs.cam_rng, &wcam = runs.wcam;
  const std::vector<hostlayout::Chunk>& chunks = runs.chunks;
  const int64_t npad = runs.npad;
  d.N_pad = npad;
  d.n_jchunks = int32_t(chunks.size());
  d.jac_blocks_rec = 8 * std::max(1, std::min((d.n_jchunks / 8 + 3) / 4, 128));
  d.jac_blocks = 8 * std::max(1, std::min((d.n_jchunks / 8 + 3) / 4, 256));
  if (const char* jw = std::getenv("SFM_JAC_WG_PER_XCD")) {
    const int v = std::atoi(jw);
    if (v > 0) d.jac_blocks = 8 * std::max(1, std::min((d.n_jchunks / 8 + 3) / 4, v));
  }
  bool small = host_check && stage_in && N > 0 && N <= kSmallSetupMaxObs && C > 0 && C <= kSmallSetupMaxC &&
               int64_t(C) * (C + 1) / 2 <= kSchurXcdMinBlocks;
  if (small) {
    const char* ss = std::getenv("SFM_SMALL_SETUP");
    if (ss && ss[0] == '0') small = false;
  }
  if (small) {
    int64_t nch_small = 0;
    for (int c = 0; c < C; ++c) nch_small += (cam_cnt[4 + c] + 63) / 64;
    small = nch_small <= kSmallSetupMaxChunks;
  }
  if (small) {
    const int32_t* pc = reinterpret_cast<const int32_t*>(stg + o_pc);
    for (int p = 0; p < P && small; ++p) small = pc[p] <= kSmallSetupMaxPtObs;
  }
  timer.mark("camera runs (host)");
  int64_t n_pairs = 0;
  int32_t *pt_s = nullptr, *cm_order = nullptr;
  const int32_t* pair_order = nullptr;
  int64_t* poff = nullptr;
  void* sort_tmp = nullptr;
  size_t sort_bytes = 0;
  int32_t* small_fill = nullptr;
  if (!small) ALLOC(d.pt_off, size_t(P) + 1);
  ALLOC(d.order, size_t(N));
  ALLOC(d.uv_pm, 2 * size_t(N));
  ALLOC(d.cam_pm, size_t(N));
  ALLOC(d.cam_obs, size_t(npad));
  ALLOC(d.cm_p, size_t(npad));
  ALLOC(d.jchunks, size_t(std::max(1, d.n_jchunks)));
  ALLOC(d.jgrp, size_t(9));
  ALLOC(d.uv_cm, 2 * size_t(npad));
  ALLOC(d.pos, size_t(N));
  uint64_t *k64a = nullptr, *k64b = nullptr;
  uint32_t *k32a = nullptr, *k32b = nullptr;
  int32_t *iota = nullptr, *d_cam_off = nullptr, *perm = nullptr;
  int4* ch_in = nullptr;
  const int64_t nch = d.n_jchunks;
  const int64_t nmax = std::max<int64_t>({N, nch, 1});
  TMP(k64a, size_t(N));
  TMP(k64b, size_t(N));
  TMP(k32a, size_t(nmax));
  TMP(k32b, size_t(nmax));
  TMP(iota, size_t(nmax));
  TMP(pt_s, size_t(N));
  TMP(cm_order, size_t(N));
  TMP(perm, size_t(std::max<int64_t>(1, nch)));
  sort_bytes = std::max({setup_sort_bytes(N, 64), setup_sort_bytes(nmax, 32), setup_sort_bytes(P + 1, 1),
                                setup_sort_bytes(N + 1, 2), size_t(256)});
  {
    uint8_t* tb = nullptr;
    TMP(tb, sort_bytes);
    sort_tmp = tb;
  }
  {
    StageLayout il;
    const size_t o_rng = il.add(sizeof(int32_t) * cam_rng.size()), o_w = il.add(sizeof(int32_t) * wcam.size()),
                 o_off = il.add(sizeof(int32_t) * cam_off.size()), o_ch = il.add(sizeof(hostlayout::Chunk) * chunks.size());
    const size_t o_poff = small ? il.add(sizeof(int32_t) * (size_t(P) + 1)) : 0,
                 o_fill = small ? il.add(sizeof(int32_t) * (size_t(P) + size_t(C))) : 0;
    if (il_base && il.bytes > il_bound) return bail(fail(SFM_EIO, "internal: camera-run blob above its bound"));
    if ((rc = stage_reserve(h, il_base + il.bytes))) return bail(rc);
    if (early_params && il_base + il.bytes > pl_base) return bail(fail(SFM_EIO, "internal: stage layout overlap"));
    stg = h->stage;
    uint8_t* ib = nullptr;
    ALLOC(ib, il.bytes);
    uint8_t* sb = stg + il_base;
    std::memcpy(sb + o_rng, cam_rng.data(), sizeof(int32_t) * cam_rng.size());
    std::memcpy(sb + o_w, wcam.data(), sizeof(int32_t) * wcam.size());
    std::memcpy(sb + o_off, cam_off.data(), sizeof(int32_t) * cam_off.size());
    if (nch) std::memcpy(sb + o_ch, chunks.data(), sizeof(hostlayout::Chunk) * chunks.size());
    if (small) {
      const int32_t* pc = reinterpret_cast<const int32_t*>(stg + o_pc);
      int32_t* po = reinterpret_cast<int32_t*>(sb + o_poff);
      po[0] = 0;
      for (int p = 0; p < P; ++p) po[p + 1] = po[p] + pc[p];
      std::memset(sb + o_fill, 0, sizeof(int32_t) * (size_t(P) + size_t(C)));
    }
    if (deferred_uv) {
      void* sbd = nullptr;
      HCHK(hipHostGetDevicePointer(&sbd, sb, 0));
      launch_copy_from_host(ib, sbd, (il.bytes + 15) / 16 * 16, s);
    } else {
      HCHK(hipMemcpyAsync(ib, sb, il.bytes, hipMemcpyHostToDevice, s));
    }
    if (small) {
      d.pt_off = reinterpret_cast<int32_t*>(ib + o_poff);
      small_fill = reinterpret_cast<int32_t*>(ib + o_fill);
    }
    d.cam_rng = reinterpret_cast<int32_t*>(ib + o_rng);
    d.wcam = reinterpret_cast<int32_t*>(ib + o_w);
    d_cam_off = reinterpret_cast<int32_t*>(ib + o_off);
    ch_in = reinterpret_cast<int4*>(ib + o_ch);
  }
  if (early_params) {
    uint8_t* pb = nullptr;
    ALLOC(pb, pl.bytes);
    d.Kc = reinterpret_cast<double*>(pb + o_K);
    d.cam = reinterpret_cast<double*>(pb + o_c);
    d.cam0 = reinterpret_cast<double*>(pb + o_c0);
    d.X = reinterpret_cast<double*>(pb + o_X);
    d.X0 = reinterpret_cast<double*>(pb + o_X0);
    uint8_t* ps = stg + pl_base;
    std::memcpy(ps + o_K, Kc.data(), sizeof(double) * Kc.size());
    std::memcpy(ps + o_c, cam.data(), sizeof(double) * cam.size());
    std::memcpy(ps + o_c0, cam.data(), sizeof(double) * cam.size());
    if (P) {
      std::memcpy(ps + o_X, X, sizeof(double) * 3 * size_t(P));
      std::memcpy(ps + o_X0, X, sizeof(double) * 3 * size_t(P));
    }
    HCHK(hipMemcpyAsync(pb, ps, pl.bytes, hipMemcpyHostToDevice, s));
  }
  int32_t* small_cnt = nullptr;
  if (small) {
    d.n_blk = int64_t(C) * (C + 1) / 2;
    ALLOC(d.seg, size_t(d.n_blk) + 1);
    TMP(small_cnt, std::max<size_t>(1, size_t(d.n_blk)));
    timer.mark("allocs + camera-run blob");
    launch_small_pm(N, in_pt, in_cam, in_uv, d.pt_off, small_fill, reinterpret_cast<int32_t*>(k32a), d.order,
                    d.uv_pm, d.cam_pm, pt_s, s);
    launch_small_cm(N, C, d.cam_pm, d_cam_off, cm_order, s);
    launch_fill_cm(npad, d.wcam, d.cam_rng, d_cam_off, cm_order, pt_s, d.uv_pm, d.cm_p, d.uv_cm, d.cam_obs, d.pos, s);
    launch_small_chunks(int(nch), ch_in, cm_order, pt_s, P, d.jchunks, d.jgrp, s);
    launch_small_pairs_count(C, d.n_blk, d_cam_off, cm_order, d.cam_pm, pt_s, d.pt_off, small_cnt, d.seg, s);
  } else {
  timer.mark("allocs + camera-run blob");
  launch_pm_keys(N, in_cam, in_pt, C, k64a, iota, s);
  HCHK(sort_pairs64(sort_tmp, sort_bytes, k64a, k64b, iota, d.order, N,
                    uint64_t(std::max(1, P)) * uint64_t(std::max(1, C)) - 1, s));
  launch_gather_pm(N, d.order, deferred_uv ? nullptr : in_uv, in_cam, in_pt, d.uv_pm, d.cam_pm, pt_s, k32a, iota, s);
  if (deferred_uv) launch_pt_off(P, k64b, N, C, d.pt_off, s);
  else HCHK(exclusive_sum32(sort_tmp, sort_bytes, cnt_p, d.pt_off, int64_t(P) + 1, s));
  HCHK(sort_pairs32(sort_tmp, sort_bytes, k32a, k32b, iota, cm_order, N, uint64_t(std::max(1, C)) - 1, s));
  launch_fill_cm(npad, d.wcam, d.cam_rng, d_cam_off, cm_order, pt_s, deferred_uv ? nullptr : d.uv_pm, d.cm_p,
                 d.uv_cm, d.cam_obs, d.pos, s);
  launch_chunk_keys(int(nch), ch_in, cm_order, pt_s, P, k32a, iota, s);
  HCHK(sort_pairs32(sort_tmp, sort_bytes, k32a, k32b, iota, perm, nch, 7, s));
  launch_chunk_gather(int(nch), perm, ch_in, k32b, d.jchunks, d.jgrp, s);
  int64_t* pcnt = nullptr;
  TMP(pcnt, size_t(N) + 1);
  TMP(poff, size_t(N) + 1);
  pair_order = env_flag("SFM_PAIRS_CM") ? cm_order : nullptr;
  launch_pair_count(N, pair_order, d.cam_pm, pt_s, d.pt_off, pcnt, s);
  HCHK(exclusive_sum64(sort_tmp, sort_bytes, pcnt, poff, N + 1, s));
  if (!deferred_uv) HCHK(hipMemcpyAsync(stg, poff + N, sizeof(int64_t), hipMemcpyDeviceToHost, s));
  }
  if (small) {
    n_pairs = std::max<int64_t>(1, 2 * pairs_est);
    d.xcd_slice_max = hostlayout::small_slice_max(C, cam_cnt.data() + 4, cam_slice);
    timer.mark("layout launches");
  } else {
    if (!deferred_uv) HCHK(hipMemcpyAsync(stg + 8, d.jgrp, 9 * sizeof(int32_t), hipMemcpyDeviceToHost, s));
    timer.mark("layout launches");
    if (deferred_uv) {
      void* stg_d = nullptr;
      HCHK(hipHostGetDevicePointer(&stg_d, stg, 0));
      uint8_t* sd = static_cast<uint8_t*>(stg_d);
      HostCopySet cs;
      cs.add(sd, poff + N, sizeof(int64_t));
      cs.add(sd + 8, d.jgrp, 9 * sizeof(int32_t));
      launch_copy_to_host(cs, s);
    }
    if (side_params && !deferred_uv) {
      if ((rc = upload_params_side())) return bail(rc);
      timer.mark("parameter upload (side stream)");
    }
    HCHK(hipStreamSynchronize(s));
    std::memcpy(&n_pairs, stg, sizeof(int64_t));
    int32_t g[9];
    std::memcpy(g, stg + 8, sizeof(g));
    d.xcd_slice_max = 0;
    for (int i = 0; i < 8; ++i) d.xcd_slice_max = std::max(d.xcd_slice_max, g[i + 1] - g[i]);
    timer.mark("layouts (device)");
  }
  if (n_pairs >= int64_t(INT32_MAX)) return bail(fail(SFM_EINVAL, "too many Schur pairs for 32-bit offsets"));
  d.n_blk = int64_t(C) * (C + 1) / 2;
  d.n_pairs = host_check && stage_in && !cam_slice.empty() ? pairs_est : n_pairs;
  if (const char* ss = std::getenv("SFM_SCHUR_PTS_SUB")) {
    const int v = std::atoi(ss);
    d.schur_pts_sub = v == 64 ? 64 : v == 32 ? 32 : v == 8 ? 8 : 16;
  } else {
    const double avg = d.n_blk ? double(d.n_pairs) / double(d.n_blk) : 0.0;
    int sub = 8;
    while (sub < 64 && sub < avg / 10.0) sub *= 2;
    d.schur_pts_sub = sub;
  }
  d.schur_wg_blocks = d.schur_pts_sub == 64 && d.n_blk <= 4 * 256 &&
                      (d.n_blk ? double(d.n_pairs) / double(d.n_blk) : 0.0) >= 256.0;
  if (const char* sw = std::getenv("SFM_SCHUR_WG")) d.schur_wg_blocks = sw[0] == '1' && d.schur_pts_sub == 64;
  if (!d.scal_host && hipHostMalloc(&d.scal_host, sizeof(double) * (kNumScalars + 1 + 17)) != hipSuccess) {
    d.scal_host = nullptr;
    return bail(fail(SFM_ENOMEM, "hipHostMalloc failed"));
  }
  int64_t* grp_host = reinterpret_cast<int64_t*>(d.scal_host + kNumScalars + 1);
  int32_t* uv_err_host = reinterpret_cast<int32_t*>(grp_host + 16);
  int bperm_per = 0;
  ALLOC(d.blk, std::max<size_t>(1, size_t(d.n_blk)));
  if (!small) ALLOC(d.seg, size_t(d.n_blk) + 1);
  ALLOC(d.bpts, std::max<size_t>(1, size_t(n_pairs)));
  if (small) {
    launch_small_pairs_fill(C, d.n_blk, d_cam_off, cm_order, d.cam_pm, pt_s, d.pt_off, d.seg, d.bpts, s);
    launch_blk(C, d.blk, s);
    d.bperm = nullptr;
    d.n_bslots = d.n_blk;
  } else {
    uint32_t *bk_a = nullptr, *bk_b = nullptr;
    int32_t* bv = nullptr;
    const int64_t nk = std::max<int64_t>({n_pairs, d.n_blk, 1});
    TMP(bk_a, size_t(nk));
    TMP(bk_b, size_t(nk));
    TMP(bv, size_t(nk));
    const size_t need = std::max(setup_sort_bytes(n_pairs, 32), setup_sort_bytes(d.n_blk, 32));
    if (need > sort_bytes) {
      uint8_t* tb = nullptr;
      TMP(tb, need);
      sort_tmp = tb;
      sort_bytes = need;
    }
    launch_pair_fill(N, pair_order, d.cam_pm, pt_s, d.pt_off, poff, C, bk_a, bv, s);
    HCHK(sort_pairs32(sort_tmp, sort_bytes, bk_a, bk_b, bv, d.bpts, n_pairs, uint64_t(std::max<int64_t>(1, d.n_blk)) - 1,
                      s));
    launch_seg(d.n_blk, bk_b, n_pairs, d.seg, s);
    launch_blk(C, d.blk, s);
    d.bperm = nullptr;
    d.n_bslots = d.n_blk;
    if (d.n_blk > kSchurXcdMinBlocks) {
      const int per = 64 / d.schur_pts_sub * (kThreads / 64);
      int32_t *sorted = nullptr, *row_x = nullptr;
      int64_t* grp = nullptr;
      TMP(sorted, size_t(d.n_blk));
      TMP(row_x, size_t(C));
      TMP(grp, 16);
      ALLOC(d.bperm, size_t(bperm_slots_bound(d.n_blk, per)));
      HCHK(launch_bperm(C, d.n_blk, n_pairs, d.seg, d.blk, per, bk_a, bk_b, bv, sorted, row_x, grp, sort_tmp,
                        sort_bytes, d.bperm, s));
      HCHK(hipMemcpyAsync(grp_host, grp, sizeof(int64_t) * 16, hipMemcpyDeviceToHost, s));
      bperm_per = per;
    }
  }
  d.n = 6 * C;
  d.ld = ((d.n + 1 + kNB - 1) / kNB) * kNB;
  d.nblk = d.ld / kNB;
  d.max_blocks = std::max({1, C, blocks_for(N, 256), blocks_for(P, 256), d.jac_blocks,
                           d.jac_blocks_rec, blocks_for(npad, 256), obs_xcd_blocks(d), pt_xcd_blocks(d)});
  if (!early_params && !side_params) {
    uint8_t* pb = nullptr;
    ALLOC(pb, pl.bytes);
    d.Kc = reinterpret_cast<double*>(pb + o_K);
    d.cam = reinterpret_cast<double*>(pb + o_c);
    d.cam0 = reinterpret_cast<double*>(pb + o_c0);
    d.X = reinterpret_cast<double*>(pb + o_X);
    d.X0 = reinterpret_cast<double*>(pb + o_X0);
  }
  ALLOC(d.cam_new, 6 * size_t(C));
  ALLOC(d.X_new, 3 * size_t(P));
  ALLOC(d.scale_c, 6 * size_t(C));
  ALLOC(d.scale_p, 3 * size_t(P));
  ALLOC(d.diag_c, 6 * size_t(C));
  ALLOC(d.diag_p, 3 * size_t(P));
  ALLOC(d.camR, size_t(kCamR) * C);
  ALLOC(d.camRn, 12 * size_t(C));
  {
    const char* ec = std::getenv("SFM_EU_CM");
    d.eu_cm = !(ec && ec[0] == '0');
  }
  ALLOC(d.eu, size_t(kEU) * size_t(d.eu_cm ? npad : N));
  ALLOC(d.ypt, 3 * size_t(P));
  ALLOC(d.ptV, size_t(kPtV) * P);
  ALLOC(d.ptL, size_t(kPtL) * P);
  ALLOC(d.ptS, size_t(kPtS) * std::max(1, P));
  ALLOC(d.Ucam, size_t(kUcam) * C);
  ALLOC(d.jpart, 27 * std::max<size_t>(1, size_t(npad / 64)));
  ALLOC(d.dpart, 27 * std::max<size_t>(1, size_t(npad / 64)));
  ALLOC(d.S, size_t(d.ld) * d.ld);
  h->force_pack = env_flag("SFM_FORCE_PACK");
  if (sharded(h) || h->force_pack) ALLOC(d.Spack, packed_size(d.n));
  ALLOC(d.invL, size_t(d.nblk) * kNB * kNB);
  ALLOC(d.flags, size_t(d.nblk));
  ALLOC(d.cflags, 2 * size_t(d.nblk) * d.nblk);
  ALLOC(d.cticket, 5);
  {
    const char* ov = std::getenv("SFM_OVERLAP");
    const int v = ov ? std::atoi(ov) : 0;
    d.overlap = v > 0 && d.nblk > 2 && !sharded(h) ? 1 : 0;
  }
  if (d.overlap) {
    ALLOC(d.tile_cnt, size_t(d.nblk) * d.nblk);
    ALLOC(d.tile_exp, size_t(d.nblk) * d.nblk);
    std::vector<int32_t> te(size_t(d.nblk) * d.nblk, 0);
    for (int c1 = 0; c1 < C; ++c1)
      for (int c2 = c1; c2 < C; ++c2)
        for (int I = 6 * c2 / kNB; I <= (6 * c2 + 5) / kNB; ++I)
          for (int J = 6 * c1 / kNB; J <= (6 * c1 + 5) / kNB; ++J) ++te[size_t(I) * d.nblk + J];
    HCHK(hipMemcpy(d.tile_exp, te.data(), sizeof(int32_t) * te.size(), hipMemcpyHostToDevice));
  }
  ALLOC(d.ysol, size_t(d.ld));
  ALLOC(d.fail, size_t(1));
  ALLOC(d.partials, size_t(kNumPartialSlots) * d.max_blocks);
  ALLOC(d.scal, size_t(kNumScalars) + 1);
#undef ALLOC
#undef TMP
  release_pool(h);
  if (deferred_uv) {
    uv_worker.join();
    if (uv_state.load(std::memory_order_acquire) != 1) return bail(fail(SFM_EIO, "observation upload failed"));
    timer.mark("uv upload (worker)");
    hipStream_t u = h->ustream;
    launch_uv_layout(N, npad, d.order, d.wcam, d.cam_rng, d_cam_off, cm_order, in_uv, d.uv_pm, d.uv_cm, err, u);
    void* ue_d = nullptr;
    HCHK(hipHostGetDevicePointer(&ue_d, uv_err_host, 0));
    HostCopySet cs;
    cs.add(ue_d, err + 2, sizeof(int32_t));
    launch_copy_to_host(cs, u);
    HCHK(hipEventRecord(h->uev_uv, u));
  }
  if (side_params) {
    if (small && (rc = upload_params_side())) return bail(rc);
    if (deferred_uv && param_state.load(std::memory_order_acquire) != 1)
      return bail(fail(SFM_EIO, "parameter upload failed"));
    HCHK(hipStreamWaitEvent(s, h->uev, 0));
  } else if ((C || P) && !early_params) {
    if (pl.bytes <= kStageMaxBytes) {
      if ((rc = stage_reserve(h, pl.bytes))) return bail(rc);
      uint8_t* ps = h->stage;
      std::memcpy(ps + o_K, Kc.data(), sizeof(double) * Kc.size());
      std::memcpy(ps + o_c, cam.data(), sizeof(double) * cam.size());
      std::memcpy(ps + o_c0, cam.data(), sizeof(double) * cam.size());
      if (P) {
        std::memcpy(ps + o_X, X, sizeof(double) * 3 * size_t(P));
        std::memcpy(ps + o_X0, X, sizeof(double) * 3 * size_t(P));
      }
      HCHK(hipMemcpyAsync(d.Kc, ps, pl.bytes, hipMemcpyHostToDevice, s));
    } else {
      HCHK(hipMemcpyAsync(d.Kc, Kc.data(), sizeof(double) * Kc.size(), hipMemcpyHostToDevice, s));
      HCHK(hipMemcpyAsync(d.cam, cam.data(), sizeof(double) * cam.size(), hipMemcpyHostToDevice, s));
      HCHK(hipMemcpyAsync(d.cam0, d.cam, sizeof(double) * cam.size(), hipMemcpyDeviceToDevice, s));
      if (P) {
        HCHK(hipMemcpyAsync(d.X, X, sizeof(double) * 3 * size_t(P), hipMemcpyHostToDevice, s));
        HCHK(hipMemcpyAsync(d.X0, d.X, sizeof(double) * 3 * size_t(P), hipMemcpyDeviceToDevice, s));
      }
    }
  }
  {
    Fill32Set fs;
    fs.add(d.S, sizeof(double) * size_t(d.ld) * d.ld, 0);
    fs.add(d.invL, sizeof(double) * size_t(d.nblk) * kNB * kNB, 0);
    fs.add(d.flags, sizeof(int32_t) * size_t(d.nblk), 0);
    fs.add(d.cflags, sizeof(int32_t) * 2 * size_t(d.nblk) * d.nblk, 0);
    fs.add(d.cticket, 5 * sizeof(unsigned long long), 0);
    fs.add(d.partials, sizeof(double) * size_t(kNumPartialSlots) * d.max_blocks, 0);
    launch_fill32(fs, s);
  }
  h->chol_epoch = 0;
  h->bs_epoch = 0;
  d.n_cu = h->n_cu;
  timer.mark("pairs + params launches");
  static const bool sync_setup = env_flag("SFM_SYNC_SETUP");
  if (deferred_uv) HCHK(hipStreamWaitEvent(s, h->uev_uv, 0));
  if (!(small && early_params && !bperm_per) || sync_setup) {
    HCHK(hipStreamSynchronize(s));
    if (deferred_uv && *uv_err_host != INT32_MAX)
      return bail(fail(SFM_EINVAL, "non-finite observation at " + std::to_string(*uv_err_host)));
    if (bperm_per) {
      int64_t m_max = 1;
      for (int x = 0; x < 8; ++x) m_max = std::max<int64_t>(m_max, (grp_host[8 + x] + bperm_per - 1) / bperm_per);
      d.n_bslots = m_max * 8 * bperm_per;
    }
    retire_tmps(h);
    timer.mark("pair lists + uploads (device)");
  }
#undef HCHK
  h->has_problem = true;
  return 0;
}

int sfm_ba_reset_parameters(sfm_ba_handle* h) {
  if (!h || !h->has_problem) return fail(SFM_EINVAL, "no problem set");
  HIPCHK(hipSetDevice(h->device));
  HIPCHK(hipMemcpyAsync(h->d.cam, h->d.cam0, sizeof(double) * 6 * size_t(h->d.C), hipMemcpyDeviceToDevice, h->stream));
  HIPCHK(hipMemcpyAsync(h->d.X, h->d.X0, sizeof(double) * 3 * size_t(h->d.P), hipMemcpyDeviceToDevice, h->stream));
  return 0;
}

int sfm_ba_get_parameters(sfm_ba_handle* h, double* rot, double* t, double* X) {
  if (!h || !h->has_problem) return fail(SFM_EINVAL, "no problem set");
  HIPCHK(hipSetDevice(h->device));
  const DevProblem& d = h->d;
  HIPCHK(hipStreamSynchronize(h->stream));
  StageLayout gl;
  const size_t o_c = gl.add(sizeof(double) * 6 * size_t(d.C)), o_X = gl.add(sizeof(double) * 3 * size_t(d.P));
  const bool stage_x = gl.bytes <= kStageMaxBytes;
  if (int rc = stage_reserve(h, stage_x ? gl.bytes : o_X)) return rc;
  const double* cam = reinterpret_cast<const double*>(h->stage + o_c);
  if (d.C) HIPCHK(hipMemcpyAsync(h->stage + o_c, d.cam, sizeof(double) * 6 * size_t(d.C), hipMemcpyDeviceToHost, h->stream));
  if (X && d.P)
    HIPCHK(hipMemcpyAsync(stage_x ? static_cast<void*>(h->stage + o_X) : static_cast<void*>(X), d.X,
                          sizeof(double) * 3 * size_t(d.P), hipMemcpyDeviceToHost, h->stream));
  HIPCHK(hipStreamSynchronize(h->stream));
  if (X && d.P && stage_x) std::memcpy(X, h->stage + o_X, sizeof(double) * 3 * size_t(d.P));
  for (int c = 0; c < d.C; ++c)
    for (int j = 0; j < 3; ++j) {
      if (rot) rot[3 * c + j] = cam[6 * c + j];
      if (t) t[3 * c + j] = cam[6 * c + 3 + j];
    }
  return 0;
}

int sfm_ba_set_profiling(sfm_ba_handle* h, int32_t on) {
  if (!h) return fail(SFM_EINVAL, "handle is NULL");
  h->profiling = on != 0;
  for (int i = 0; i < kNumPh; ++i) { h->phase_ms[i] = 0; h->phase_count[i] = 0; }
  return 0;
}

int sfm_ba_phase_times(sfm_ba_handle* h, double* ms) {
  if (!h || !ms) return fail(SFM_EINVAL, "bad arguments");
  for (int i = 0; i < kNumPh; ++i) ms[i] = h->phase_ms[i];
  for (int i = 0; i < kNumPh; ++i) ms[kNumPh + i] = h->phase_count[i];
  return 0;
}

int sfm_ba_sync(sfm_ba_handle* h) {
  if (!h) return fail(SFM_EINVAL, "handle is NULL");
  HIPCHK(hipSetDevice(h->device));
  HIPCHK(hipStreamSynchronize(h->stream));
  return 0;
}

int sfm_ba_solve_resident(sfm_ba_handle* h, const sfm_ba_options* opts_in, int32_t mode, sfm_ba_summary* summary,
                          sfm_ba_iteration* trace, int32_t trace_cap, int32_t* trace_len) {
  SFM_TRACE("sfm_ba_solve_resident");
  const auto t_start = std::chrono::steady_clock::now();
  auto now_s = [&]() { return std::chrono::duration<double>(std::chrono::steady_clock::now() - t_start).count(); };
  if (!h || !h->has_problem) return fail(SFM_EINVAL, "no problem set");
  sfm_ba_options opts;
  if (opts_in) opts = *opts_in; else sfm_ba_default_options(&opts);
  if (const char* why = invalid_option(opts)) return fail(SFM_EINVAL, std::string("invalid option: ") + why);
  sfm_ba_summary sm;
  std::memset(&sm, 0, sizeof(sm));
  int tl = 0;
  if (trace_len) *trace_len = 0;
  auto push = [&](const sfm_ba_iteration& it) {
    if (trace && tl < trace_cap) trace[tl] = it;
    ++tl;
    if (trace_len) *trace_len = std::min(tl, trace_cap);
  };
  if (mode < 0 || mode > 2 || h->d.N == 0) {
    sm.termination_type = SFM_CONVERGENCE;
    if (summary) *summary = sm;
    return 0;
  }
  HIPCHK(hipSetDevice(h->device));
  DevProblem& d = h->d;
  h->mode = mode;
  d.min_diag = opts.min_lm_diagonal;
  d.max_diag = opts.max_lm_diagonal;
  int rc;
  if (!opts.jacobi_scaling) {
    std::vector<double> ones(std::max(6 * size_t(d.C), 3 * size_t(d.P)), 1.0);
    HIPCHK(hipMemcpyAsync(d.scale_c, ones.data(), sizeof(double) * 6 * d.C, hipMemcpyHostToDevice, h->stream));
    if (d.P) HIPCHK(hipMemcpyAsync(d.scale_p, ones.data(), sizeof(double) * 3 * d.P, hipMemcpyHostToDevice, h->stream));
  }
  if (mode == SFM_BA_STRUCT_ONLY && d.C) HIPCHK(hipMemsetAsync(d.scale_c, 0, sizeof(double) * 6 * d.C, h->stream));
  if (mode == SFM_BA_POSE_ONLY && d.P) HIPCHK(hipMemsetAsync(d.scale_p, 0, sizeof(double) * 3 * d.P, h->stream));
  double* sc = d.scal_host;
  if (!h->host_fn && !h->coll_fn && !(sharded(h) && h->dist_pt > 0) && !env_flag("SFM_HOST_LM")) {
    double cost = 0.0;
    bool nonfinite = false;
    rc = run_device_lm(h, opts, &cost, &sm, push, &nonfinite);
    if (rc) {
      if (nonfinite && summary) *summary = sm;
      return rc;
    }
    sm.final_cost = cost;
    sm.wall_time_s = now_s();
    if (summary) *summary = sm;
    return 0;
  }
  double tj = now_s();
  if ((rc = evaluate(h, true, opts.jacobi_scaling != 0))) return rc;
  sm.jacobian_time_s += now_s() - tj;
  sm.num_jacobian_evaluations++;
  sm.num_residual_evaluations++;
  double cost = sc[kCost];
  sm.initial_cost = cost;
  if (!std::isfinite(cost)) {
    sm.termination_type = SFM_FAILURE;
    sm.final_cost = cost;
    if (summary) *summary = sm;
    return fail(SFM_EIO, "initial residual evaluation is not finite");
  }
  double grad_max = std::max(sc[kGradMaxCam], sc[kGradMaxPt]);
  double x_norm = std::sqrt(sc[kXNorm2Cam] + sc[kXNorm2Pt]);
  {
    sfm_ba_iteration it0;
    std::memset(&it0, 0, sizeof(it0));
    it0.cost = cost;
    it0.gradient_max_norm = grad_max;
    it0.trust_region_radius = opts.initial_trust_region_radius;
    it0.step_is_valid = 1;
    it0.step_is_successful = 1;
    push(it0);
  }
  if (grad_max <= opts.gradient_tolerance) {
    sm.termination_type = SFM_CONVERGENCE;
  } else {
    double radius = opts.initial_trust_region_radius;
    double decrease_factor = 2.0;
    int num_consecutive_invalid = 0;
    int iteration = 0;
    while (true) {
      if (iteration >= opts.max_num_iterations) { sm.termination_type = SFM_NO_CONVERGENCE; break; }
      ++iteration;
      sfm_ba_iteration itr;
      std::memset(&itr, 0, sizeof(itr));
      itr.iteration = iteration;
      const double tls = now_s();
      if ((rc = compute_step(h, radius))) return rc;
      sm.linear_solver_time_s += now_s() - tls;
      sm.num_linear_solves++;
      int chol_fail = 0;
      std::memcpy(&chol_fail, sc + kNumScalars, sizeof(int));
      if (chol_fail & 4) return fail(SFM_EIO, "Cholesky tile hand-off timed out (persistent grid made no progress)");
      if (chol_fail & 2) return fail(SFM_EIO, "back-substitution hand-off timed out (persistent grid made no progress)");
      const bool solve_ok = chol_fail == 0 && !(sc[kBadStep] > 0.0) && !(sc[kBadCam] > 0.0) && !(sc[kBadBack] > 0.0);
      const double model_cost_change = sc[kModelChange] + sc[kModelChangePt];
      itr.step_is_valid = (solve_ok && model_cost_change >= 0.0) ? 1 : 0;
      itr.step_is_successful = 0;
      if (!itr.step_is_valid) {
        ++num_consecutive_invalid;
        sm.num_invalid_steps++;
        if (num_consecutive_invalid >= opts.max_num_consecutive_invalid_steps) {
          sm.termination_type = SFM_FAILURE;
          itr.cost = cost; itr.gradient_max_norm = grad_max; itr.trust_region_radius = radius;
          push(itr);
          break;
        }
        itr.cost = cost;
        itr.gradient_max_norm = grad_max;
      } else {
        num_consecutive_invalid = 0;
        double new_cost = sc[kNewCost];
        if (!std::isfinite(new_cost)) new_cost = std::numeric_limits<double>::max();
        sm.num_residual_evaluations++;
        itr.step_norm = std::sqrt(sc[kStep2Cam] + sc[kStep2Pt]);
        const double step_size_tolerance = opts.parameter_tolerance * (x_norm + opts.parameter_tolerance);
        if (itr.step_norm <= step_size_tolerance) {
          sm.termination_type = SFM_CONVERGENCE;
          itr.cost = cost; itr.gradient_max_norm = grad_max; itr.trust_region_radius = radius;
          push(itr);
          break;
        }
        itr.cost_change = cost - new_cost;
        if (std::fabs(itr.cost_change) <= opts.function_tolerance * cost) {
          sm.termination_type = SFM_CONVERGENCE;
          itr.cost = cost; itr.gradient_max_norm = grad_max; itr.trust_region_radius = radius;
          push(itr);
          break;
        }
        itr.relative_decrease = itr.cost_change / model_cost_change;
        itr.step_is_successful = itr.relative_decrease > opts.min_relative_decrease;
      }
      if (itr.step_is_successful) {
        sm.num_successful_steps++;
        const double q = 2.0 * itr.relative_decrease - 1.0;
        radius = radius / std::max(1.0 / 3.0, 1.0 - q * q * q);
        radius = std::min(opts.max_trust_region_radius, radius);
        decrease_factor = 2.0;
        std::swap(d.cam, d.cam_new);
        std::swap(d.X, d.X_new);
        tj = now_s();
        if ((rc = evaluate(h, false, opts.jacobi_scaling != 0))) return rc;
        sm.jacobian_time_s += now_s() - tj;
// ... 329 lines not shown
```

Baseline: 1.661 billion residual-evals/s (obs x evaluations).

## Factor camera rotation out of Schur pair kernel and add point-major backsubstitution

The point factor kernel now also writes a per-point record: the position plus the scaled inverse Cholesky factor. A new Schur off-diagonal kernel uses it to accumulate 6x6 blocks in a rotation-free frame with cross products, then applies each camera's rotation Jacobian once per block instead of once per observation. Camera staging is vectorised across lanes, and a first-order fast path is used when a camera's rotation derivatives equal the skew basis. Separately, a point-major backsubstitution kernel fuses the point solve, the update and the new-cost evaluation, reading cameras from a small precomputed table (at most 512 cameras); this adds extra buffers and a larger accumulator footprint per thread.

After: 1.786 billion residual-evals/s (obs x evaluations) (median of 6 runs). 1.08x the previous value.

```diff
diff --git a/sfm_amd/csrc/ba_device.h b/sfm_amd/csrc/ba_device.h
--- a/sfm_amd/csrc/ba_device.h
+++ b/sfm_amd/csrc/ba_device.h
@@ -10,9 +10,12 @@
 constexpr int kEU = 4;
 constexpr int kCamR = 36;
 constexpr int kUcam = 28;
+constexpr int kCamPM = 37;
+constexpr int kCamPMMax = 512;
 constexpr int kPtV = 10;
 constexpr int kPtL = 10;
 constexpr int kPtS = 16;
+constexpr int kPtG = 16;
 constexpr int kNB = 64;
 constexpr int kThreads = 256;
 constexpr uint32_t kYSentinelWord = 0x7FF4DEADu;
@@ -78,6 +81,7 @@
   double* diag_p = nullptr;
   double* camR = nullptr;
   double* camRn = nullptr;
+  double* campm = nullptr;
   double* jrec = nullptr;
   double* eu = nullptr;
   bool eu_cm = false;
@@ -105,6 +109,7 @@
   int32_t* bperm = nullptr;
   int64_t n_bslots = 0;
   double* ptS = nullptr;
+  double* ptG = nullptr;
   int32_t schur_pts_sub = 8;
   bool schur_wg_blocks = false;
   double* dpart = nullptr;
@@ -140,7 +145,10 @@
 void launch_pad_init(const DevProblem& d, hipStream_t s);
 void launch_pack_upper(const DevProblem& d, bool unpack, hipStream_t s);
 void launch_gated_copy(const double* src, double* dst, int64_t n, double scale, const int32_t* gate, hipStream_t s);
-void launch_cam_update(const DevProblem& d, bool count_norm, hipStream_t s);
+void launch_cam_update(const DevProblem& d, bool count_norm, hipStream_t s, bool pm = false);
+inline bool backsub_pm(const DevProblem& d, bool cams_var, bool pts_var) {
+  return d.campm && cams_var && pts_var && d.P > 0 && d.N_pad > 0;
+}
 bool launch_point_eval_with_cams(const DevProblem& d, int mode, bool count_grad, hipStream_t s);
 void launch_point_backsub(const DevProblem& d, hipStream_t s, bool cams_var = true, bool pts_var = true);
 inline int obs_xcd_blocks(const DevProblem& d) {
diff --git a/sfm_amd/csrc/ba_kernels.hip b/sfm_amd/csrc/ba_kernels.hip
--- a/sfm_amd/csrc/ba_kernels.hip
+++ b/sfm_amd/csrc/ba_kernels.hip
@@ -448,7 +448,8 @@
                                                            double* __restrict__ ptL, double* __restrict__ part_bad,
                                                            const double* __restrict__ X,
                                                            const double* __restrict__ scale_p,
-                                                           double* __restrict__ ptS, const int* __restrict__ gate, const double* __restrict__ radius_dev) {
+                                                           double* __restrict__ ptS, const int* __restrict__ gate, const double* __restrict__ radius_dev,
+                                                           double* __restrict__ ptG) {
   if (gate && *gate == 0) return;
   if (radius_dev) radius = *radius_dev;
   __shared__ double sh[4];
@@ -476,6 +477,15 @@
       st2(o + 6, l10, l20); st2(o + 8, l21, 1.0 / l00); st2(o + 10, 1.0 / l11, 1.0 / l22);
       st2(o + 12, z0, z1); st2(o + 14, z2, 0.0);
     }
+    if (ptG) {
+      const double* x = X + 3 * size_t(p);
+      const double* sp = scale_p + 3 * size_t(p);
+      const double i00 = 1.0 / l00, i11 = 1.0 / l11, i22 = 1.0 / l22;
+      const double li10 = -l10 * i00 * i11, li21 = -l21 * i11 * i22, li20 = -(l20 * i00 + l21 * li10) * i22;
+      double* o = ptG + size_t(kPtG) * p;
+      st2(o, x[0], x[1]); st2(o + 2, x[2], sp[0] * i00); st2(o + 4, sp[0] * li10, sp[0] * li20);
+      st2(o + 6, sp[1] * i11, sp[1] * li21); st2(o + 8, sp[2] * i22, 0.0);
+    }
   }
   const double r = block_reduce(bad, sh, true);
   if (threadIdx.x == 0) part_bad[blockIdx.x] = r;
@@ -920,20 +930,100 @@
   }
 }
 
-template <int kSub, int kHalf>
-__global__ __launch_bounds__(kThreads, 4) void k_schur_pts_half(int64_t n_slots, const int2* __restrict__ blk,
-                                                             const int32_t* __restrict__ seg,
-                                                             const int32_t* __restrict__ bpts,
-                                                             const double* __restrict__ ptS,
-                                                             const double* __restrict__ camR,
-                                                             const double* __restrict__ cam,
-                                                             const double* __restrict__ Kc,
-                                                             const double* __restrict__ scale_c, double* __restrict__ S,
-                                                             int ld, const int32_t* __restrict__ bperm,
-                                                             const int* __restrict__ gate) {
-  if (gate && *gate == 0) return;
+__device__ __forceinline__ double skew_basis_entry(int k, int i) {
+  const int r = i / 3, q = i % 3;
+  return (r == (k + 2) % 3 && q == (k + 1) % 3) ? 1.0 : (r == (k + 1) % 3 && q == (k + 2) % 3) ? -1.0 : 0.0;
+}
+constexpr int kCamSR = 32;
+
+template <int kSub>
+__device__ __forceinline__ void stage_cams_rot(double* cs_wave, int cx, int cy, const double* __restrict__ camR,
+                                               const double* __restrict__ cam, const double* __restrict__ Kc,
+                                               const double* __restrict__ scale_c, int l) {
   constexpr int kPer = 64 / kSub;
-  __shared__ __attribute__((aligned(16))) double cst[kThreads / 64][kPer][2 * kCamS];
+  const int q = l % kPer, j = l / kPer;
+  bool ok0 = true, ok1 = true;
+#pragma unroll
+  for (int idx0 = 0; idx0 < 54; idx0 += kSub) {
+    const int idx = min(idx0 + j, 53);
+    const int side = idx >= 27, en = idx - 27 * side;
+    const bool ok = camR[size_t(kCamR) * (side ? cy : cx) + 9 + en] == skew_basis_entry(en / 9, en % 9);
+    ok0 = ok0 & (bool(side) | ok);
+    ok1 = ok1 & (!side | ok);
+  }
+  unsigned long long mask = 0;
+#pragma unroll
+  for (int t = 0; t < kSub; ++t) mask |= 1ull << (kPer * t);
+  mask <<= q;
+  const bool fo0 = (__ballot(ok0) & mask) == mask, fo1 = (__ballot(ok1) & mask) == mask;
+#pragma unroll
+  for (int i0 = 0; i0 < 64; i0 += kSub) {
+    const int i = i0 + j, side = i >> 5, hl = i & 31;
+    const int c = side ? cy : cx;
+    const bool fo = side ? fo1 : fo0;
+    const double* cr = camR + size_t(kCamR) * c;
+    const int e = min(max(hl - 16, 0), 8);
+    const int r = e / 3, k = e % 3, a = (r + 2) % 3, b = (r + 1) % 3;
+    const double* D = cr + 9 + 9 * k;
+    const bool round_has_j = kSub >= 32 || ((i0 & 31) + kSub - 1 >= 16 && (i0 & 31) <= 24);
+    double wab = 0.0, wba = 0.0;
+    if (round_has_j) {
+      wab = D[3 * a] * cr[3 * b] + D[3 * a + 1] * cr[3 * b + 1] + D[3 * a + 2] * cr[3 * b + 2];
+      wba = D[3 * b] * cr[3 * a] + D[3 * b + 1] * cr[3 * a + 1] + D[3 * b + 2] * cr[3 * a + 2];
+    }
+    asm("" : "+v"(wab), "+v"(wba));
+    double jv = fo ? (r == k ? 1.0 : 0.0) : 0.5 * (wab - wba);
+    const double* src = hl < 9 ? cr + hl
+                      : hl < 12 ? cam + 6 * size_t(c) + 3 + (hl - 9)
+                      : hl < 15 ? Kc + 5 * size_t(c) + (hl == 14 ? 3 : hl - 12)
+                      : (hl >= 25 && hl < 31) ? scale_c + 6 * size_t(c) + (hl - 25) : cr;
+    asm("" : "+v"(src));
+    double pv = *src;
+    asm("" : "+v"(jv), "+v"(pv));
+    const double v = hl == 15 ? (fo ? 1.0 : 0.0) : (hl >= 16 && hl < 25) ? jv : pv;
+    if (hl < 31) cs_wave[(2 * q + side) * kCamSR + hl] = v;
+  }
+}
+
+__device__ __forceinline__ void pair_side_rot(const double* cs, const double Xp[3], const double G[6], double y[3],
+                                              double M[6], double ab[5]) {
+  const double fx = cs[12], sk = cs[13], fy = cs[14];
+  const double y0 = cs[0] * Xp[0] + cs[1] * Xp[1] + cs[2] * Xp[2];
+  const double y1 = cs[3] * Xp[0] + cs[4] * Xp[1] + cs[5] * Xp[2];
+  const double y2 = cs[6] * Xp[0] + cs[7] * Xp[1] + cs[8] * Xp[2];
+  const double pc0 = y0 + cs[9], pc1 = y1 + cs[10], pc2 = y2 + cs[11];
+  const double iz = srcp(shared_div(pc2)), xp = pc0 * iz, yp = pc1 * iz;
+  const double a0 = fx * iz, a1 = sk * iz, a2 = -(fx * xp + sk * yp) * iz;
+  const double b1 = fy * iz, b2 = -fy * yp * iz;
+  ab[0] = a0; ab[1] = a1; ab[2] = a2; ab[3] = b1; ab[4] = b2;
+  const bool fo = cs[15] != 0.0;
+  y[0] = fo ? Xp[0] : y0; y[1] = fo ? Xp[1] : y1; y[2] = fo ? Xp[2] : y2;
+  double e[6];
+#pragma unroll
+  for (int j = 0; j < 3; ++j) {
+    e[j] = a0 * cs[j] + a1 * cs[3 + j] + a2 * cs[6 + j];
+    e[3 + j] = b1 * cs[3 + j] + b2 * cs[6 + j];
+  }
+  M[0] = e[0] * G[0]; M[1] = e[0] * G[1] + e[1] * G[3]; M[2] = e[0] * G[2] + e[1] * G[4] + e[2] * G[5];
+  M[3] = e[3] * G[0]; M[4] = e[3] * G[1] + e[4] * G[3]; M[5] = e[3] * G[2] + e[4] * G[4] + e[5] * G[5];
+}
+
+template <int kSub>
+__global__ __launch_bounds__(kThreads, 2) void k_schur_pairs_rot(int64_t n_slots, const int2* __restrict__ blk,
+                                                              const int32_t* __restrict__ seg,
+                                                              const int32_t* __restrict__ bpts,
+                                                              const double* __restrict__ ptG,
+                                                              const double* __restrict__ camR,
+                                                              const double* __restrict__ cam,
+                                                              const double* __restrict__ Kc,
+                                                              const double* __restrict__ scale_c,
+                                                              double* __restrict__ S, int ld,
+                                                              const int32_t* __restrict__ bperm,
+                                                              const int* __restrict__ gate, int* __restrict__ tile_cnt,
+                                                              int nbt) {
+  if (gate && *gate == 0) return;
+  constexpr int kPer = 64 / kSub;
+  __shared__ __attribute__((aligned(16))) double cst[kThreads / 64][kPer][2 * kCamSR];
   const int l = threadIdx.x & 63, wv = threadIdx.x >> 6, g = l / kSub, sl = l % kSub;
   const int64_t wb = (int64_t(blockIdx.x) * (kThreads / 64) + wv) * kPer;
   auto slot_blk = [&](int64_t k) -> int32_t { return k < n_slots ? (bperm ? bperm[k] : int32_t(k)) : -1; };
@@ -941,42 +1031,45 @@
   const bool own = bs >= 0;
   const int64_t b = own ? bs : 0;
   const int2 cc = blk[b];
-  double* cs1 = cst[wv][g];
-  double* cs2 = cs1 + kCamS;
-#pragma unroll
-  for (int q = 0; q < kPer; ++q) {
-    const int32_t bq = slot_blk(wb + q);
+  const double* cs1 = cst[wv][g];
+  const double* cs2 = cs1 + kCamSR;
+  {
+    const int32_t bq = slot_blk(wb + l % kPer);
     const int2 cq = blk[bq >= 0 ? bq : 0];
-    stage_cam(cst[wv][q], cq.x, camR, cam, Kc, scale_c, l);
-    stage_cam(cst[wv][q] + kCamS, cq.y, camR, cam, Kc, scale_c, l);
+    stage_cams_rot<kSub>(&cst[wv][0][0], cq.x, cq.y, camR, cam, Kc, scale_c, l);
   }
   wave_lds_sync();
   const int kb = seg[b], ke = own ? seg[b + 1] : kb;
-  double acc[18];
-#pragma unroll
-  for (int e = 0; e < 18; ++e) acc[e] = 0.0;
+  double acc[36];
+#pragma unroll
+  for (int e = 0; e < 36; ++e) acc[e] = 0.0;
   int len = ke - kb;
 #pragma unroll
   for (int off = kSub; off < 64; off <<= 1) len = max(len, __shfl_xor(len, off));
-  int p_nx = bpts[kb + sl < ke ? kb + sl : 0];
+  int p_nx = bpts[kb + sl + kSub < ke ? kb + sl + kSub : 0];
+  double2 n0, n1, n2, n3, n4;
+  {
+    const double* r = ptG + size_t(kPtG) * bpts[kb + sl < ke ? kb + sl : 0];
+    n0 = ld2(r); n1 = ld2(r + 2); n2 = ld2(r + 4); n3 = ld2(r + 6); n4 = ld2(r + 8);
+  }
   for (int k0 = 0; k0 < len; k0 += kSub) {
-    asm volatile("" ::: "memory");
+    double2 x0 = n0, x1 = n1, x2 = n2, x3 = n3, x4 = n4;
+    asm volatile("" : "+v"(x0.x), "+v"(x0.y), "+v"(x1.x), "+v"(x1.y), "+v"(x2.x), "+v"(x2.y), "+v"(x3.x), "+v"(x3.y),
+                 "+v"(x4.x), "+v"(p_nx));
     const int k = kb + k0 + sl;
     const bool valid = k < ke;
-    const int p = p_nx;
-    p_nx = bpts[k + kSub < ke ? k + kSub : 0];
-    const double* r = ptS + size_t(kPtS) * p;
-    double q[12];
-#pragma unroll
-    for (int f = 0; f < 12; f += 2) {
-      const double2 x = ld2(r + f);
-      q[f] = x.x; q[f + 1] = x.y;
-    }
-    const double Xp[3] = {q[0], q[1], q[2]}, sp[3] = {q[3], q[4], q[5]};
-    const double Lp[6] = {q[6], q[7], q[8], q[9], q[10], q[11]};
-    double M1[6], ab1[5], M2[6], ab2[5];
-    pair_side_m(cs1, Xp, sp, Lp, M1, ab1);
-    pair_side_m(cs2, Xp, sp, Lp, M2, ab2);
+    {
+      const double* r = ptG + size_t(kPtG) * p_nx;
+      n0 = ld2(r); n1 = ld2(r + 2); n2 = ld2(r + 4); n3 = ld2(r + 6); n4 = ld2(r + 8);
+    }
+    p_nx = bpts[k + 2 * kSub < ke ? k + 2 * kSub : 0];
+    asm volatile("" ::: "memory");
+    const double Xp[3] = {x0.x, x0.y, x1.x};
+    const double G[6] = {x1.y, x2.x, x2.y, x3.x, x3.y, x4.x};
+    double M1[6], ab1[5], y1[3], M2[6], ab2[5], y2[3];
+    pair_side_rot(cs1, Xp, G, y1, M1, ab1);
+    asm volatile("" ::: "memory");
+    pair_side_rot(cs2, Xp, G, y2, M2, ab2);
     asm volatile("" ::: "memory");
     const double w = valid ? 1.0 : 0.0;
     const double g00 = (M1[0] * M2[0] + M1[1] * M2[1] + M1[2] * M2[2]) * w;
@@ -991,60 +1084,75 @@
       H[1][0] = ab1[1] * t00 + ab1[3] * t10; H[1][1] = ab1[1] * t01 + ab1[3] * t11; H[1][2] = ab1[1] * t02 + ab1[3] * t12;
       H[2][0] = ab1[2] * t00 + ab1[4] * t10; H[2][1] = ab1[2] * t01 + ab1[4] * t11; H[2][2] = ab1[2] * t02 + ab1[4] * t12;
     }
-    double HQ[3][3];
-#pragma unroll
-    for (int kq = 0; kq < 3; ++kq) {
-      const double* D = cs2 + 9 + 9 * kq;
-      const double q0 = D[0] * Xp[0] + D[1] * Xp[1] + D[2] * Xp[2];
-      const double q1 = D[3] * Xp[0] + D[4] * Xp[1] + D[5] * Xp[2];
-      const double q2 = D[6] * Xp[0] + D[7] * Xp[1] + D[8] * Xp[2];
-#pragma unroll
-      for (int i = 0; i < 3; ++i) HQ[i][kq] = H[i][0] * q0 + H[i][1] * q1 + H[i][2] * q2;
-    }
-    if (kHalf == 0) {
-#pragma unroll
-      for (int u = 0; u < 3; ++u) {
-        const double* D = cs1 + 9 + 9 * u;
-        const double q0 = D[0] * Xp[0] + D[1] * Xp[1] + D[2] * Xp[2];
-        const double q1 = D[3] * Xp[0] + D[4] * Xp[1] + D[5] * Xp[2];
-        const double q2 = D[6] * Xp[0] + D[7] * Xp[1] + D[8] * Xp[2];
-#pragma unroll
-        for (int v = 0; v < 3; ++v) {
-          acc[6 * u + v] += q0 * HQ[0][v] + q1 * HQ[1][v] + q2 * HQ[2][v];
-          acc[6 * u + 3 + v] += q0 * H[0][v] + q1 * H[1][v] + q2 * H[2][v];
-        }
-      }
-    } else {
-#pragma unroll
-      for (int u = 0; u < 3; ++u)
-#pragma unroll
-        for (int v = 0; v < 3; ++v) {
-          acc[6 * u + v] += HQ[u][v];
-          acc[6 * u + 3 + v] += H[u][v];
-        }
+    double Kx[3][3];
+#pragma unroll
+    for (int v = 0; v < 3; ++v) {
+      Kx[0][v] = y1[1] * H[2][v] - y1[2] * H[1][v];
+      Kx[1][v] = y1[2] * H[0][v] - y1[0] * H[2][v];
+      Kx[2][v] = y1[0] * H[1][v] - y1[1] * H[0][v];
+    }
+#pragma unroll
+    for (int u = 0; u < 3; ++u) {
+      acc[6 * u + 0] += y2[1] * Kx[u][2] - y2[2] * Kx[u][1];
+      acc[6 * u + 1] += y2[2] * Kx[u][0] - y2[0] * Kx[u][2];
+      acc[6 * u + 2] += y2[0] * Kx[u][1] - y2[1] * Kx[u][0];
+      acc[6 * u + 3] += Kx[u][0]; acc[6 * u + 4] += Kx[u][1]; acc[6 * u + 5] += Kx[u][2];
+      acc[6 * (3 + u) + 0] += y2[1] * H[u][2] - y2[2] * H[u][1];
+      acc[6 * (3 + u) + 1] += y2[2] * H[u][0] - y2[0] * H[u][2];
+      acc[6 * (3 + u) + 2] += y2[0] * H[u][1] - y2[1] * H[u][0];
+      acc[6 * (3 + u) + 3] += H[u][0]; acc[6 * (3 + u) + 4] += H[u][1]; acc[6 * (3 + u) + 5] += H[u][2];
+    }
+  }
+  {
+    const double* J1 = cs1 + 16;
+    const double* J2 = cs2 + 16;
+#pragma unroll
+    for (int v = 0; v < 6; ++v) {
+      const double a0 = acc[v], a1 = acc[6 + v], a2 = acc[12 + v];
+#pragma unroll
+      for (int k = 0; k < 3; ++k) acc[6 * k + v] = J1[k] * a0 + J1[3 + k] * a1 + J1[6 + k] * a2;
+    }
+#pragma unroll
+    for (int u = 0; u < 6; ++u) {
+      const double a0 = acc[6 * u], a1 = acc[6 * u + 1], a2 = acc[6 * u + 2];
+#pragma unroll
+      for (int k = 0; k < 3; ++k) acc[6 * u + k] = a0 * J2[k] + a1 * J2[3 + k] + a2 * J2[6 + k];
     }
   }
   double v32[32];
 #pragma unroll
-  for (int e = 0; e < 32; ++e) v32[e] = e < 18 ? acc[e] : 0.0;
+  for (int e = 0; e < 32; ++e) v32[e] = acc[e];
   seg_reduce32<kSub>(v32, l);
+  const double t32 = seg_sum<kSub>(acc[32]), t33 = seg_sum<kSub>(acc[33]), t34 = seg_sum<kSub>(acc[34]),
+               t35 = seg_sum<kSub>(acc[35]);
   if (own) {
     double* Sb = S + size_t(6 * cc.x) * ld + 6 * size_t(cc.y);
     const bool add = cc.x == cc.y;
-    const double* sc1 = cst[wv][g] + 44;
-    const double* sc2 = sc1 + kCamS;
+    const double* sc1 = cs1 + 25;
+    const double* sc2 = cs2 + 25;
     auto put = [&](int e, double v) {
       double* q = Sb + size_t(e / 6) * ld + e % 6;
       v = v * sc1[e / 6] * sc2[e % 6];
-      *q = add ? *q - v : -v;
+      v = add ? *q - v : -v;
+      if (tile_cnt) __hip_atomic_store(q, v, __ATOMIC_RELAXED, __HIP_MEMORY_SCOPE_AGENT);
+      else *q = v;
     };
     constexpr int kR = kSub >= 32 ? 1 : 32 / kSub;
     if (kSub == 64) {
-      if (!(sl & 1) && (sl >> 1) < 18) put(18 * kHalf + (sl >> 1), v32[0]);
+      if (!(sl & 1)) put(sl >> 1, v32[0]);
     } else {
 #pragma unroll
-      for (int r = 0; r < kR; ++r)
-        if (kR * sl + r < 18) put(18 * kHalf + kR * sl + r, v32[r]);
+      for (int r = 0; r < kR; ++r) put(kR * sl + r, v32[r]);
+    }
+    if (sl < 4) put(32 + sl, sl == 0 ? t32 : sl == 1 ? t33 : sl == 2 ? t34 : t35);
+  }
+  if (tile_cnt) {
+    asm volatile("s_waitcnt vmcnt(0)" ::: "memory");
+    if (own && sl == 0) {
+      const int r0 = 6 * cc.y, c0 = 6 * cc.x;
+      for (int I = r0 / 64; I <= (r0 + 5) / 64; ++I)
+        for (int J = c0 / 64; J <= (c0 + 5) / 64; ++J)
+          __hip_atomic_fetch_add(tile_cnt + I * nbt + J, 1, __ATOMIC_RELAXED, __HIP_MEMORY_SCOPE_AGENT);
     }
   }
 }
@@ -1096,16 +1204,56 @@
   if (j == n && threadIdx.x == 0) S[size_t(n) * ld + n] = 1.0;
 }
 
+__device__ __forceinline__ void cam_pm_pack(int c, const double* __restrict__ camR, const double* __restrict__ cam,
+                                            const double* __restrict__ Kc, const double* __restrict__ ysol,
+                                            const double* __restrict__ scale_c, const double* camRn,
+                                            double* __restrict__ campm) {
+  const double* cr = camR + size_t(kCamR) * c;
+  double* o = campm + size_t(kCamPM) * c;
+  double R[9], sy[6];
+  for (int i = 0; i < 9; ++i) R[i] = cr[i];
+  for (int k = 0; k < 6; ++k) sy[k] = scale_c[6 * c + k] * ysol[6 * c + k];
+  bool first_order = true;
+#pragma unroll
+  for (int k = 0; k < 3; ++k)
+#pragma unroll
+    for (int i = 0; i < 9; ++i)
+      first_order = first_order & (cr[9 + 9 * k + i] == skew_basis_entry(k, i));
+  double om[3] = {sy[0], sy[1], sy[2]};
+  if (!first_order) {
+    om[0] = om[1] = om[2] = 0.0;
+    for (int k = 0; k < 3; ++k) {
+      const double* D = cr + 9 + 9 * k;
+      double W[9];
+      for (int i = 0; i < 3; ++i)
+        for (int j = 0; j < 3; ++j) W[3 * i + j] = D[3 * i] * R[3 * j] + D[3 * i + 1] * R[3 * j + 1] + D[3 * i + 2] * R[3 * j + 2];
+      om[0] += 0.5 * (W[7] - W[5]) * sy[k];
+      om[1] += 0.5 * (W[2] - W[6]) * sy[k];
+      om[2] += 0.5 * (W[3] - W[1]) * sy[k];
+    }
+  }
+  for (int i = 0; i < 9; ++i) o[i] = R[i];
+  for (int i = 0; i < 3; ++i) o[9 + i] = cam[6 * c + 3 + i];
+  for (int i = 0; i < 5; ++i) o[12 + i] = Kc[5 * size_t(c) + i];
+  for (int i = 0; i < 3; ++i) { o[17 + i] = om[i]; o[20 + i] = sy[3 + i]; }
+  for (int i = 0; i < 12; ++i) o[23 + i] = camRn[12 * size_t(c) + i];
+  o[35] = first_order ? 1.0 : 0.0;
+  o[36] = 0.0;
+}
+
 __global__ __launch_bounds__(kThreads) void k_cam_update(int C, const double* __restrict__ cam,
                                                          const double* __restrict__ ysol,
                                                          const double* __restrict__ scale_c,
                                                          double* __restrict__ cam_new, double* __restrict__ camRn,
-                                                         double* __restrict__ part_step, double* __restrict__ part_bad, const int* __restrict__ gate) {
+                                                         double* __restrict__ part_step, double* __restrict__ part_bad, const int* __restrict__ gate,
+                                                         const double* __restrict__ camR, const double* __restrict__ Kc,
+                                                         double* __restrict__ campm) {
   if (gate && *gate == 0) return;
   __shared__ double sh[4];
   const int c = blockIdx.x * blockDim.x + threadIdx.x;
   double st = 0.0, bad = 0.0;
   if (c < C) cam_update_one(c, cam, ysol, scale_c, cam_new, camRn, st, bad);
+  if (c < C && campm) cam_pm_pack(c, camR, cam, Kc, ysol, scale_c, camRn, campm);
   const double rs = block_reduce(st, sh, false);
   if (threadIdx.x == 0 && part_step) part_step[blockIdx.x] = rs;
   const double rb = block_reduce(bad, sh, true);
@@ -1274,6 +1422,122 @@
   }
   const double r = block_reduce(ncost, sh, false);
   if (threadIdx.x == 0) part_cost[blockIdx.x] = r;
+}
+
+template <int kGroups>
+__global__ __launch_bounds__(kThreads * kGroups) void k_backsub_pm(
+    int P, int C, const int32_t* __restrict__ pt_off, const int32_t* __restrict__ cam_pm,
+    const double* __restrict__ uv_pm, const double* __restrict__ campm, const double* __restrict__ ptL,
+    const double* __restrict__ ptV, const double* __restrict__ scale_p, const double* __restrict__ X,
+    double* __restrict__ X_new, double* __restrict__ ypt, double* __restrict__ part_model,
+    double* __restrict__ part_model_pt, double* __restrict__ part_step, double* __restrict__ part_bad,
+    double* __restrict__ part_cost, const int* __restrict__ gate) {
+  if (gate && *gate == 0) return;
+  __shared__ double sh[4 * kGroups];
+  __shared__ double cst[kCamPMMax * kCamPM];
+  for (int i = threadIdx.x; i < C * kCamPM; i += blockDim.x) cst[i] = campm[i];
+  __syncthreads();
+  const int nbp = (P + kThreads - 1) / kThreads;
+  const int grp = int(threadIdx.x) / kThreads, tg = int(threadIdx.x) % kThreads;
+  const int vb = int(blockIdx.x) * kGroups + grp;
+  const int p = vb * kThreads + tg;
+  double model = 0.0, model_pt = 0.0, st = 0.0, bad = 0.0, ncost = 0.0;
+  if (p < P) {
+    const double Xp[3] = {X[3 * size_t(p)], X[3 * size_t(p) + 1], X[3 * size_t(p) + 2]};
+    const double sp[3] = {scale_p[3 * size_t(p)], scale_p[3 * size_t(p) + 1], scale_p[3 * size_t(p) + 2]};
+    const int q0 = pt_off[p], q1 = pt_off[p + 1];
+    int c_n = q0 < q1 ? cam_pm[q0] : 0;
+    double2 uv_n = q0 < q1 ? ld2(uv_pm + 2 * size_t(q0)) : make_double2(0.0, 0.0);
+    double h0 = 0.0, h1 = 0.0, h2 = 0.0;
+    for (int q = q0; q < q1; ++q) {
+      const double* k = cst + kCamPM * c_n;
+      const double2 uvo = uv_n;
+      if (q + 1 < q1) {
+        c_n = cam_pm[q + 1];
+        uv_n = ld2(uv_pm + 2 * size_t(q + 1));
+      }
+      const double y0 = k[0] * Xp[0] + k[1] * Xp[1] + k[2] * Xp[2];
+      const double y1 = k[3] * Xp[0] + k[4] * Xp[1] + k[5] * Xp[2];
+      const double y2 = k[6] * Xp[0] + k[7] * Xp[1] + k[8] * Xp[2];
+      const double pc0 = y0 + k[9], pc1 = y1 + k[10], pc2 = y2 + k[11];
+      const double fx = k[12], sk = k[13], cx = k[14], fy = k[15], cy = k[16];
+      const double iz = srcp(shared_div(pc2)), xp = pc0 * iz, yp = pc1 * iz;
+      const double r0 = fx * xp + sk * yp + cx - uvo.x;
+      const double r1 = fy * yp + cy - uvo.y;
+      const double a0 = fx * iz, a1 = sk * iz, a2 = -(fx * xp + sk * yp) * iz;
+      const double b1 = fy * iz, b2 = -fy * yp * iz;
+      const bool fo = k[35] != 0.0;
+      const double t0 = fo ? Xp[0] : y0, t1 = fo ? Xp[1] : y1, t2 = fo ? Xp[2] : y2;
+      const double d0 = k[18] * t2 - k[19] * t1 + k[20];
+      const double d1 = k[19] * t0 - k[17] * t2 + k[21];
+      const double d2 = k[17] * t1 - k[18] * t0 + k[22];
+      const double e0 = a0 * d0 + a1 * d1 + a2 * d2, e1 = b1 * d1 + b2 * d2;
+      model += e0 * r0 + e1 * r1 - 0.5 * (e0 * e0 + e1 * e1);
+      h0 += ((a0 * k[0] + a1 * k[3] + a2 * k[6]) * e0 + (b1 * k[3] + b2 * k[6]) * e1) * sp[0];
+      h1 += ((a0 * k[1] + a1 * k[4] + a2 * k[7]) * e0 + (b1 * k[4] + b2 * k[7]) * e1) * sp[1];
+      h2 += ((a0 * k[2] + a1 * k[5] + a2 * k[8]) * e0 + (b1 * k[5] + b2 * k[8]) * e1) * sp[2];
+    }
+    const double* L = ptL + size_t(kPtL) * p;
+    const double l00 = L[0], l10 = L[1], l11 = L[2], l20 = L[3], l21 = L[4], l22 = L[5];
+    const double s0 = h0 / l00, s1 = (h1 - l10 * s0) / l11, s2 = (h2 - l20 * s0 - l21 * s1) / l22;
+    const double w0 = L[6] - s0, w1 = L[7] - s1, w2 = L[8] - s2;
+    const double yp2 = w2 / l22;
+    const double yp1 = (w1 - l21 * yp2) / l11;
+    const double yp0 = (w0 - l10 * yp1 - l20 * yp2) / l00;
+    if (!isfinite(yp0) || !isfinite(yp1) || !isfinite(yp2)) bad = 1.0;
+    {
+      const double* v = ptV + size_t(kPtV) * p;
+      const double yVy = v[0] * yp0 * yp0 + v[2] * yp1 * yp1 + v[5] * yp2 * yp2 +
+                         2.0 * (v[1] * yp0 * yp1 + v[3] * yp0 * yp2 + v[4] * yp1 * yp2);
+      model_pt = yp0 * (v[6] - h0) + yp1 * (v[7] - h1) + yp2 * (v[8] - h2) - 0.5 * yVy;
+    }
+    const double ys[3] = {yp0, yp1, yp2};
+    double Xn[3];
+#pragma unroll
+    for (int j = 0; j < 3; ++j) {
+      Xn[j] = Xp[j] + sp[j] * (-ys[j]);
+      const double dd = Xp[j] - Xn[j];
+      st += dd * dd;
+      X_new[3 * size_t(p) + j] = Xn[j];
+      ypt[3 * size_t(p) + j] = ys[j];
+    }
+    c_n = q0 < q1 ? cam_pm[q0] : 0;
+    uv_n = q0 < q1 ? ld2(uv_pm + 2 * size_t(q0)) : make_double2(0.0, 0.0);
+    for (int q = q0; q < q1; ++q) {
+      const double* k = cst + kCamPM * c_n;
+      const double2 uvo = uv_n;
+      if (q + 1 < q1) {
+        c_n = cam_pm[q + 1];
+        uv_n = ld2(uv_pm + 2 * size_t(q + 1));
+      }
+      const double* Rn = k + 23;
+      double pc[3];
+#pragma unroll
+      for (int j = 0; j < 3; ++j) pc[j] = Rn[3 * j] * Xn[0] + Rn[3 * j + 1] * Xn[1] + Rn[3 * j + 2] * Xn[2] + Rn[9 + j];
+      const SharedDiv dz = shared_div(pc[2]);
+      const double xp = sdiv(dz, pc[0]), ypj = sdiv(dz, pc[1]);
+      const double rn0 = k[12] * xp + k[13] * ypj + k[14] - uvo.x;
+      const double rn1 = k[15] * ypj + k[16] - uvo.y;
+      ncost += 0.5 * (rn0 * rn0 + rn1 * rn1);
+    }
+  }
+  const int w = int(threadIdx.x) >> 6, l = int(threadIdx.x) & 63;
+  auto group_reduce = [&](double v, bool is_max, double* __restrict__ part) {
+    v = is_max ? wave_max(v) : wave_sum(v);
+    __syncthreads();
+    if (l == 0) sh[w] = v;
+    __syncthreads();
+    if (tg == 0 && vb < nbp) {
+      double r = sh[4 * grp];
+      for (int i = 1; i < 4; ++i) r = is_max ? fmax(r, sh[4 * grp + i]) : r + sh[4 * grp + i];
+      part[vb] = r;
+    }
+  };
+  group_reduce(model, false, part_model);
+  group_reduce(model_pt, false, part_model_pt);
+  group_reduce(st, false, part_step);
+  group_reduce(bad, true, part_bad);
+  group_reduce(ncost, false, part_cost);
 }
 
 __global__ __launch_bounds__(1024) void k_reduce_batch(const double* __restrict__ partials, int64_t max_blocks,
@@ -1374,7 +1638,8 @@
 }
 void launch_point_factor(const DevProblem& d, double radius, hipStream_t s) {
   if (d.P) k_point_factor<<<blocks_for(d.P, kThreads), kThreads, 0, s>>>(d.P, d.ptV, d.diag_p, radius, d.ptL,
-                                                                         slot(d, kPBad), d.X, d.scale_p, d.ptS, d.gate, d.radius_dev);
+                                                                         slot(d, kPBad), d.X, d.scale_p, d.ptS, d.gate, d.radius_dev,
+                                                                         d.ptG);
 }
 void launch_point_prep(const DevProblem& d, double radius, hipStream_t s) {
   launch_point_factor(d, radius, s);
@@ -1415,19 +1680,15 @@
                                                                     bperm, d.gate, tile_cnt, d.nblk, DiagFold{});
     return;
   }
-  static const bool halves = [] {
-    const char* e = std::getenv("SFM_SCHUR_HALVES");
-    return e && e[0] == '1';
-  }();
-  if (halves && !tile_cnt) {
-#define SFM_PTS_H(S_, H_)                                                                                       \
-  k_schur_pts_half<S_, H_><<<nb, kThreads, 0, s>>>(n_slots, d.blk, d.seg, d.bpts, d.ptS, d.camR, d.cam, d.Kc, \
-                                                   d.scale_c, d.S, d.ld, bperm, d.gate)
-    if (sub == 8) { SFM_PTS_H(8, 0); SFM_PTS_H(8, 1); }
-    else if (sub == 16) { SFM_PTS_H(16, 0); SFM_PTS_H(16, 1); }
-    else if (sub == 32) { SFM_PTS_H(32, 0); SFM_PTS_H(32, 1); }
-    else { SFM_PTS_H(64, 0); SFM_PTS_H(64, 1); }
-#undef SFM_PTS_H
+  if (d.ptG) {
+#define SFM_ROT(S_)                                                                                              \
+  k_schur_pairs_rot<S_><<<nb, kThreads, 0, s>>>(n_slots, d.blk, d.seg, d.bpts, d.ptG, d.camR, d.cam, d.Kc, d.scale_c, \
+                                                d.S, d.ld, bperm, d.gate, tile_cnt, d.nblk)
+    if (sub == 8) SFM_ROT(8);
+    else if (sub == 16) SFM_ROT(16);
+    else if (sub == 32) SFM_ROT(32);
+    else SFM_ROT(64);
+#undef SFM_ROT
     return;
   }
   if (sub == 8) SFM_PTS(8);
@@ -1450,16 +1711,24 @@
   const int n_y = (d.n + kNB - 1) / kNB * kNB;
   k_pad_init<<<d.ld, 64, 0, s>>>(d.S, d.ld, d.n, d.fail, reinterpret_cast<unsigned long long*>(d.ysol), n_y, d.gate);
 }
-void launch_cam_update(const DevProblem& d, bool count_norm, hipStream_t s) {
+void launch_cam_update(const DevProblem& d, bool count_norm, hipStream_t s, bool pm) {
   k_cam_update<<<blocks_for(d.C, kThreads), kThreads, 0, s>>>(d.C, d.cam, d.ysol, d.scale_c, d.cam_new, d.camRn,
                                                              count_norm ? slot(d, kPStepCam) : nullptr,
-                                                             slot(d, kPBadCam), d.gate);
+                                                             slot(d, kPBadCam), d.gate, d.camR, d.Kc,
+                                                             pm ? d.campm : nullptr);
 }
 void launch_cam_solve(const DevProblem& d, double radius, hipStream_t s) {
   (void)hipMemsetAsync(d.fail, 0, sizeof(int), s);
   if (d.C) k_cam_solve<<<blocks_for(d.C, kThreads), kThreads, 0, s>>>(d.C, d.Ucam, d.diag_c, radius, d.ysol, d.fail, d.gate, d.radius_dev);
 }
 void launch_point_backsub(const DevProblem& d, hipStream_t s, bool cams_var, bool pts_var) {
+  if (backsub_pm(d, cams_var, pts_var)) {
+    constexpr int kG = 4;
+    k_backsub_pm<kG><<<blocks_for(d.P, kG * kThreads), kG * kThreads, 0, s>>>(
+        d.P, d.C, d.pt_off, d.cam_pm, d.uv_pm, d.campm, d.ptL, d.ptV, d.scale_p, d.X, d.X_new, d.ypt,
+        slot(d, kPModel), slot(d, kPModelPt), slot(d, kPStepPt), slot(d, kPBadBack), slot(d, kPNewCost), d.gate);
+    return;
+  }
   if (d.N_pad && cams_var)
     k_backsub_a_rc<<<obs_xcd_blocks(d), kThreads, 0, s>>>(d.jgrp, d.jchunks, d.cm_p, d.uv_cm, d.cam_obs, d.camR,
                                                           d.cam, d.Kc, d.scale_c, d.ptS, d.ysol, d.eu, d.eu_cm ? 1 : 0,
diff --git a/sfm_amd/csrc/ba_solver.hip b/sfm_amd/csrc/ba_solver.hip
--- a/sfm_amd/csrc/ba_solver.hip
+++ b/sfm_amd/csrc/ba_solver.hip
@@ -899,9 +899,11 @@
     }
     hipMemsetAsync(d.ysol, 0, sizeof(double) * 6 * size_t(d.C), s);
   }
-  if (!cam_done) launch_cam_update(d, h->rank == 0 && h->mode != SFM_BA_STRUCT_ONLY, s);
+  const bool cams_var = h->mode != SFM_BA_STRUCT_ONLY, pts_var = h->mode != SFM_BA_POSE_ONLY;
+  const bool pm = backsub_pm(d, cams_var, pts_var);
+  if (!cam_done) launch_cam_update(d, h->rank == 0 && cams_var, s, pm);
   mark_begin(h, kPhBacksub);
-  launch_point_backsub(d, s, h->mode != SFM_BA_STRUCT_ONLY, h->mode != SFM_BA_POSE_ONLY);
+  launch_point_backsub(d, s, cams_var, pts_var);
   mark_end(h);
   if (d.P == 0) {
     const int slots[] = {kPModel, kPModelPt, kPNewCost, kPStepPt, kPBadBack, kPBad};
@@ -909,8 +911,8 @@
   }
   if (h->rank != 0 || h->mode == SFM_BA_STRUCT_ONLY)
     hipMemsetAsync(d.partials + size_t(kPStepCam) * d.max_blocks, 0, sizeof(double) * nbC, s);
-  const int nbI = d.N_pad ? obs_xcd_blocks(d) : 1;
-  const int nbB = d.P ? pt_xcd_blocks(d) : 1;
+  const int nbI = pm ? nbP : d.N_pad ? obs_xcd_blocks(d) : 1;
+  const int nbB = pm ? nbP : d.P ? pt_xcd_blocks(d) : 1;
   ReduceBatch rb;
   rb.add(kPModel, nbI, 0, kModelChange);
   rb.add(kPNewCost, nbI, 0, kNewCost);
@@ -1702,6 +1704,8 @@
   ALLOC(d.diag_p, 3 * size_t(P));
   ALLOC(d.camR, size_t(kCamR) * C);
   ALLOC(d.camRn, 12 * size_t(C));
+  d.campm = nullptr;
+  if (d.n_blk > kSchurXcdMinBlocks && C <= kCamPMMax) ALLOC(d.campm, size_t(kCamPM) * C);
   {
     const char* ec = std::getenv("SFM_EU_CM");
     d.eu_cm = !(ec && ec[0] == '0');
@@ -1711,6 +1715,8 @@
   ALLOC(d.ptV, size_t(kPtV) * P);
   ALLOC(d.ptL, size_t(kPtL) * P);
   ALLOC(d.ptS, size_t(kPtS) * std::max(1, P));
+  d.ptG = nullptr;
+  if (d.n_blk > kSchurXcdMinBlocks) ALLOC(d.ptG, size_t(kPtG) * std::max(1, P));
   ALLOC(d.Ucam, size_t(kUcam) * C);
   ALLOC(d.jpart, 27 * std::max<size_t>(1, size_t(npad / 64)));
   ALLOC(d.dpart, 27 * std::max<size_t>(1, size_t(npad / 64)));
```
